# cpmech/russell

Measured on AMD Instinct MI355X. Metric: factorize+solve time (ms) + SpTRSV GB/s, 1M-DOF 5-pt Poisson f64, 1/2/4/8 GPU, lower is better.
Workload: dtype f64; 1 GPU; values+rhs resident in HBM: numeric LU factorize + solve, 2D 5-point Poisson 1000x1000 grid (n=1000000, nnz=4996000) f64, general storage, 1 RHS per GPU (through host pointers: value_host_boundary_ms); rhs_per_gpu=1, refinement_steps=1

## Files before the change

include/russell_hipmf.h:

```cpp
#ifndef RUSSELL_HIPMF_H
#define RUSSELL_HIPMF_H

#include <inttypes.h>
#include <stddef.h>

#ifdef __cplusplus
extern "C" {
#endif

#define C_BOOL int32_t

#define SUCCESSFUL_EXIT 0
#define ERROR_NULL_POINTER 100000
#define ERROR_MALLOC 200000
#define ERROR_VERSION 300000
#define ERROR_NOT_AVAILABLE 400000
#define ERROR_NEED_INITIALIZATION 500000
#define ERROR_NEED_FACTORIZATION 600000
#define ERROR_ALREADY_INITIALIZED 700000

#define HIPMF_WARNING_SINGULAR_MATRIX 1
#define ERROR_HIP_MALLOC 100
#define ERROR_HIP_MEMCPY 200
#define ERROR_HIP_SYNCHRONIZE 300
// ... 34 lines not shown

int32_t solver_hipmf_factorize(struct InterfaceHIPMF *solver,
                               int32_t *effective_ordering,
                               int32_t *effective_scaling,
                               int32_t *num_perturbed_pivots,
                               double *rcond_estimate,
                               double *determinant_coefficient,
                               double *determinant_exponent,
                               C_BOOL compute_determinant,
                               C_BOOL verbose,
                               const double *values);

int32_t solver_hipmf_solve(struct InterfaceHIPMF *solver, double *x, const double *rhs, C_BOOL verbose);


int32_t solver_hipmf_solve_many(struct InterfaceHIPMF *solver, double *x, const double *rhs, int32_t nrhs, int32_t ld,
                                C_BOOL verbose);

int32_t solver_hipmf_prepare_solve_many(struct InterfaceHIPMF *solver, int32_t nrhs);

int32_t solver_hipmf_factorize_device(struct InterfaceHIPMF *solver, const double *d_values);
int32_t solver_hipmf_solve_device(struct InterfaceHIPMF *solver, double *d_x, const double *d_rhs, int32_t nrhs, int32_t ld);

int32_t solver_hipmf_solve_transpose(struct InterfaceHIPMF *solver, double *x, const double *rhs, C_BOOL verbose);
int32_t solver_hipmf_solve_transpose_device(struct InterfaceHIPMF *solver, double *d_x, const double *d_rhs, int32_t nrhs, int32_t ld);
int32_t solver_hipmf_solve_transpose_many(struct InterfaceHIPMF *solver, double *x, const double *rhs, int32_t nrhs, int32_t ld, C_BOOL verbose);
int32_t solver_hipmf_solve_transpose_many_device(struct InterfaceHIPMF *solver, double *d_x, const double *d_rhs, int32_t nrhs, int32_t ld);

int32_t solver_hipmf_solve_sparse(struct InterfaceHIPMF *solver, double *x_sel, int32_t ldx, int32_t nrhs, const int32_t *rhs_ptr,
                                  const int32_t *rhs_idx, const double *rhs_val, int32_t nsel, const int32_t *sel_idx, C_BOOL verbose);
int32_t solver_hipmf_solve_sparse_device(struct InterfaceHIPMF *solver, double *d_x_sel, int32_t ldx, int32_t nrhs, const int32_t *d_rhs_ptr,
                                         const int32_t *d_rhs_idx, const double *d_rhs_val, int32_t nsel, const int32_t *d_sel_idx, C_BOOL verbose);
int32_t solver_hipmf_inverse_entries(struct InterfaceHIPMF *solver, int32_t nent, const int32_t *rows, const int32_t *cols, double *values, C_BOOL verbose);

int32_t solver_hipmf_solve_with_error_analysis(struct InterfaceHIPMF *solver, double *x, const double *rhs, double *error_analysis_array_len_8,
                                               int32_t error_analysis_option, C_BOOL verbose);

int32_t solver_hipmf_mat_vec_mul(struct InterfaceHIPMF *solver, double *v, double alpha, const double *u);

int32_t solver_hipmf_set_value_map(struct InterfaceHIPMF *solver, int32_t nnz_in, const int32_t *seg_ptr, const int32_t *seg_idx);
int32_t solver_hipmf_factorize_mapped(struct InterfaceHIPMF *solver, int32_t *effective_ordering, int32_t *effective_scaling,
                                      int32_t *num_perturbed_pivots, double *rcond_estimate, double *determinant_coefficient,
                                      double *determinant_exponent, C_BOOL compute_determinant, C_BOOL verbose,
                                      const double *input_values);
int32_t solver_hipmf_factorize_mapped_device(struct InterfaceHIPMF *solver, const double *d_input_values);

int32_t solver_hipmf_get_permutation(struct InterfaceHIPMF *solver, int32_t *perm);

int32_t hipmf_max_product_matching(int32_t ndim, const int32_t *row_pointers, const int32_t *col_indices, const double *values,
                                   int32_t *matched_row, double *row_scale, double *col_scale);
int32_t hipmf_paired_matching(int32_t ndim2, const int32_t *row_pointers, const int32_t *col_indices, const double *values, int32_t *matched_row,
                              double *row_scale, double *col_scale);

int32_t solver_hipmf_get_stats(struct InterfaceHIPMF *solver, int64_t *istats, double *dstats);
int32_t solver_hipmf_reset_timers(struct InterfaceHIPMF *solver);
#define HIPMF_COUNTER_REMATCH 0
#define HIPMF_COUNTER_WEAK_DIAGONAL_ROWS 1
#define HIPMF_COUNTER_FUSED_FALLBACKS 2
#define HIPMF_COUNTER_PERSISTENT_BYTES 3
#define HIPMF_COUNTER_ARENA_BYTES 4
#define HIPMF_COUNTER_SYMMETRIC_LDLT 5
#define HIPMF_COUNTER_SYM_EXPANDED 6
#define HIPMF_COUNTER_MID_FRONTS 8
#define HIPMF_COUNTER_CHAIN_FALLBACKS 7
#define HIPMF_COUNTER_PLAN_DIGEST 9
#define HIPMF_COUNTER_TAGGED_SOLVE 10
#define HIPMF_COUNTER_GATE_WAITS 11
#define HIPMF_COUNTER_WAVE_FRONTS 12
#define HIPMF_COUNTER_LEAF_FRONTS 13
#define HIPMF_COUNTER_SPLIT_SLABS 14
#define HIPMF_COUNTER_EVENT_FENCE_FREE 15
#define HIPMF_COUNTER_BLOCK_GROUPS 16
#define HIPMF_COUNTER_SYM_WEAK_DIAGONAL 17
#define HIPMF_COUNTER_BCAST_SLICED_BYTES 18
#define HIPMF_COUNTER_KRYLOV_ITERATIONS 19
#define HIPMF_COUNTER_TRANSPOSED_SOLVES 20
#define HIPMF_COUNTER_ANALYSIS_SOLVES 21
#define HIPMF_COUNTER_TRANSPOSED_KRYLOV_ITERATIONS 22
#define HIPMF_COUNTER_TRANSPOSED_BLOCKS 23
#define HIPMF_COUNTER_PRUNED_FWD_FRONTS 24
#define HIPMF_COUNTER_PRUNED_BWD_FRONTS 25
#define HIPMF_COUNTER_PRUNED_BLOCKS 26
#define HIPMF_COUNTER_PRUNED_BYTES 27
int64_t solver_hipmf_get_counter(struct InterfaceHIPMF *solver, int32_t which);

#define HIPMF_OPTION_MATCHING 0
#define HIPMF_OPTION_PIVOTING 1
#define HIPMF_OPTION_HYBRID_MEMORY 2
#define HIPMF_OPTION_ERROR_ESTIMATES 3
#define HIPMF_OPTION_CONDITION_NUMBERS 4
#define HIPMF_OPTION_SYM_RECHECK 5
#define HIPMF_OPTION_EFFECTIVE_PIVOTING 6
int32_t solver_hipmf_set_option(struct InterfaceHIPMF *solver, int32_t option, double value);
int32_t solver_hipmf_get_option(struct InterfaceHIPMF *solver, int32_t option, double *value);

#define HIPMF_COMM_ID_BYTES 128
int32_t solver_hipmf_factor_parts(struct InterfaceHIPMF *solver, int32_t max_parts, void **d_ptrs, int64_t *bytes);
int32_t hipmf_comm_unique_id(void *id128);
int32_t hipmf_comm_init_rank(void **comm, int32_t nranks, const void *id128, int32_t rank);
void hipmf_comm_destroy(void *comm);
int32_t solver_hipmf_broadcast_factor(struct InterfaceHIPMF *solver, void *comm, int32_t root, int32_t rank, double *seconds,
                                      int64_t *bytes_sent);
int32_t solver_hipmf_solve_many_sharded(struct InterfaceHIPMF *solver, double *d_x, const double *d_rhs, int32_t nrhs_total, int32_t ld,
                                        int32_t nranks, int32_t rank, int32_t *first_column, int32_t *num_columns);
int32_t solver_hipmf_adopt_factor(struct InterfaceHIPMF *solver, const double *d_values);

const char *solver_hipmf_last_error(struct InterfaceHIPMF *solver);

struct InterfaceComplexHIPMF;
struct InterfaceComplexHIPMF *complex_solver_hipmf_new(void);
void complex_solver_hipmf_drop(struct InterfaceComplexHIPMF *solver);
int32_t complex_solver_hipmf_initialize(struct InterfaceComplexHIPMF *solver, int32_t ordering, int32_t scaling, double pivot_epsilon,
                                        int32_t refinement_nstep, C_BOOL verbose, C_BOOL general_symmetric, int32_t ndim,
                                        const int32_t *row_pointers, const int32_t *col_indices, const double *values);
int32_t complex_solver_hipmf_factorize(struct InterfaceComplexHIPMF *solver, int32_t *effective_ordering, int32_t *effective_scaling,
                                       int32_t *num_perturbed_pivots, double *rcond_estimate, double *determinant_coefficient_real,
                                       double *determinant_coefficient_imag, double *determinant_exponent, C_BOOL compute_determinant, C_BOOL verbose,
                                       const double *values);
int32_t complex_solver_hipmf_get_determinant(struct InterfaceComplexHIPMF *solver, double *determinant_coefficient_real,
                                             double *determinant_coefficient_imag, double *determinant_exponent);
int32_t complex_solver_hipmf_solve(struct InterfaceComplexHIPMF *solver, double *x, const double *rhs, C_BOOL verbose);
int32_t complex_solver_hipmf_solve_transpose(struct InterfaceComplexHIPMF *solver, double *x, const double *rhs, int32_t conjugate, C_BOOL verbose);
int32_t complex_solver_hipmf_solve_with_error_analysis(struct InterfaceComplexHIPMF *solver, double *x, const double *rhs, double *error_analysis_array_len_8,
                                                       int32_t error_analysis_option, C_BOOL verbose);
int32_t complex_solver_hipmf_set_value_map(struct InterfaceComplexHIPMF *solver, int32_t nnz_in, const int32_t *seg_ptr, const int32_t *seg_idx);
int32_t complex_solver_hipmf_factorize_mapped(struct InterfaceComplexHIPMF *solver, int32_t *effective_ordering, int32_t *effective_scaling,
                                              int32_t *num_perturbed_pivots, double *rcond_estimate, C_BOOL verbose, const double *input_values);
int32_t complex_solver_hipmf_get_stats(struct InterfaceComplexHIPMF *solver, int64_t *istats, double *dstats);
int64_t complex_solver_hipmf_get_counter(struct InterfaceComplexHIPMF *solver, int32_t which);
const char *complex_solver_hipmf_last_error(struct InterfaceComplexHIPMF *solver);

void *hipmf_device_malloc(size_t bytes);
void hipmf_device_free(void *ptr);
int32_t hipmf_memcpy_h2d(void *dst, const void *src, size_t bytes);
int32_t hipmf_memcpy_d2h(void *dst, const void *src, size_t bytes);
int32_t hipmf_device_synchronize(void);
int32_t hipmf_device_count(void);
int32_t hipmf_device_mem_info(size_t *free_bytes, size_t *total_bytes);
int32_t hipmf_device_copy_bandwidth(int64_t bytes, int32_t reps, double *gb_per_s);
int32_t hipmf_device_mfma_rate(int32_t workgroups, int32_t iters, double *tflops);
int32_t hipmf_set_device(int32_t device);

void *hipmf_fdm_new(int32_t nx, int32_t ny, int32_t nz, int32_t periodic_x, int32_t periodic_y, int32_t periodic_z, int32_t sym,
                    const uint8_t *prescribed);
void hipmf_fdm_drop(void *fdm);
int32_t hipmf_fdm_dims(const void *fdm, int64_t *nu, int64_t *np, int64_t *nnz_bar, int64_t *nnz_check);
int32_t hipmf_fdm_structure_device(const void *fdm, int32_t *d_bar_i, int32_t *d_bar_j, int32_t *d_check_i, int32_t *d_check_j);
int32_t hipmf_fdm_values_device(const void *fdm, double dx, double dy, double dz, double kx, double ky, double kz, double alpha,
                                double *d_bar_values, double *d_check_values);
int32_t hipmf_fdm_lmm_dims(void *fdm, int64_t *neq, int64_t *nlag, int64_t *nnz);
int32_t hipmf_fdm_lmm_structure_device(void *fdm, int32_t *d_i, int32_t *d_j);
int32_t hipmf_fdm_lmm_values_device(void *fdm, double dx, double dy, double dz, double kx, double ky, double kz, double alpha, double *d_values);

#ifdef __cplusplus
}
#endif
#endif
```

russell_amd/_capi.py:

```python
import ctypes as C
import os

import numpy as np

_HERE = os.path.dirname(os.path.abspath(__file__))
DEFAULT_LIB = os.path.join(_HERE, "lib", "librussell_hipmf.so")

i32p = np.ctypeslib.ndpointer(dtype=np.int32, flags="C_CONTIGUOUS")
i64p = np.ctypeslib.ndpointer(dtype=np.int64, flags="C_CONTIGUOUS")
f64p = np.ctypeslib.ndpointer(dtype=np.float64, flags="C_CONTIGUOUS")

SYMBOLS = {
    "solver_hipmf_new": (C.c_void_p, []),
    "solver_hipmf_drop": (None, [C.c_void_p]),
    "solver_hipmf_initialize": (C.c_int32, [C.c_void_p, C.c_int32, C.c_int32, C.c_double, C.c_int32, C.c_int32, C.c_int32,
                                            C.c_int32, C.c_int32, i32p, i32p, C.c_void_p]),
    "solver_hipmf_factorize": (C.c_int32, [C.c_void_p, C.POINTER(C.c_int32), C.POINTER(C.c_int32), C.POINTER(C.c_int32),
                                           C.POINTER(C.c_double), C.POINTER(C.c_double), C.POINTER(C.c_double), C.c_int32,
                                           C.c_int32, f64p]),
    "solver_hipmf_solve": (C.c_int32, [C.c_void_p, f64p, f64p, C.c_int32]),
    "solver_hipmf_solve_many": (C.c_int32, [C.c_void_p, f64p, f64p, C.c_int32, C.c_int32, C.c_int32]),
    "solver_hipmf_prepare_solve_many": (C.c_int32, [C.c_void_p, C.c_int32]),
    "solver_hipmf_factorize_device": (C.c_int32, [C.c_void_p, C.c_void_p]),
    "solver_hipmf_solve_device": (C.c_int32, [C.c_void_p, C.c_void_p, C.c_void_p, C.c_int32, C.c_int32]),
    "solver_hipmf_solve_transpose": (C.c_int32, [C.c_void_p, f64p, f64p, C.c_int32]),
    "solver_hipmf_solve_transpose_device": (C.c_int32, [C.c_void_p, C.c_void_p, C.c_void_p, C.c_int32, C.c_int32]),
    "solver_hipmf_solve_transpose_many": (C.c_int32, [C.c_void_p, f64p, f64p, C.c_int32, C.c_int32, C.c_int32]),
    "solver_hipmf_solve_transpose_many_device": (C.c_int32, [C.c_void_p, C.c_void_p, C.c_void_p, C.c_int32, C.c_int32]),
    "solver_hipmf_solve_sparse": (C.c_int32, [C.c_void_p, f64p, C.c_int32, C.c_int32, i32p, i32p, f64p, C.c_int32, C.c_void_p, C.c_int32]),
    "solver_hipmf_solve_sparse_device": (C.c_int32, [C.c_void_p, C.c_void_p, C.c_int32, C.c_int32, C.c_void_p, C.c_void_p, C.c_void_p, C.c_int32,
                                                      C.c_void_p, C.c_int32]),
    "solver_hipmf_inverse_entries": (C.c_int32, [C.c_void_p, C.c_int32, i32p, i32p, f64p, C.c_int32]),
    "solver_hipmf_solve_with_error_analysis": (C.c_int32, [C.c_void_p, f64p, f64p, f64p, C.c_int32, C.c_int32]),
    "solver_hipmf_mat_vec_mul": (C.c_int32, [C.c_void_p, f64p, C.c_double, f64p]),
    "solver_hipmf_get_permutation": (C.c_int32, [C.c_void_p, i32p]),
    "solver_hipmf_set_value_map": (C.c_int32, [C.c_void_p, C.c_int32, i32p, i32p]),
    "solver_hipmf_factorize_mapped": (C.c_int32, [C.c_void_p, C.POINTER(C.c_int32), C.POINTER(C.c_int32), C.POINTER(C.c_int32),
                                                  C.POINTER(C.c_double), C.POINTER(C.c_double), C.POINTER(C.c_double), C.c_int32,
                                                  C.c_int32, f64p]),
    "solver_hipmf_factorize_mapped_device": (C.c_int32, [C.c_void_p, C.c_void_p]),
    "hipmf_max_product_matching": (C.c_int32, [C.c_int32, i32p, i32p, f64p, i32p, f64p, f64p]),
    "hipmf_paired_matching": (C.c_int32, [C.c_int32, i32p, i32p, f64p, i32p, f64p, f64p]),
    "solver_hipmf_get_stats": (C.c_int32, [C.c_void_p, i64p, f64p]),
    "solver_hipmf_reset_timers": (C.c_int32, [C.c_void_p]),
    "complex_solver_hipmf_new": (C.c_void_p, []),
    "complex_solver_hipmf_drop": (None, [C.c_void_p]),
    "complex_solver_hipmf_initialize": (C.c_int32, [C.c_void_p, C.c_int32, C.c_int32, C.c_double, C.c_int32, C.c_int32, C.c_int32, C.c_int32,
                                                     i32p, i32p, C.c_void_p]),
    "complex_solver_hipmf_factorize": (C.c_int32, [C.c_void_p, C.POINTER(C.c_int32), C.POINTER(C.c_int32), C.POINTER(C.c_int32),
                                                    C.POINTER(C.c_double), C.POINTER(C.c_double), C.POINTER(C.c_double), C.POINTER(C.c_double),
                                                    C.c_int32, C.c_int32, f64p]),
    "complex_solver_hipmf_get_determinant": (C.c_int32, [C.c_void_p, C.POINTER(C.c_double), C.POINTER(C.c_double), C.POINTER(C.c_double)]),
    "complex_solver_hipmf_solve": (C.c_int32, [C.c_void_p, f64p, f64p, C.c_int32]),
    "complex_solver_hipmf_solve_transpose": (C.c_int32, [C.c_void_p, f64p, f64p, C.c_int32, C.c_int32]),
    "complex_solver_hipmf_solve_with_error_analysis": (C.c_int32, [C.c_void_p, f64p, f64p, f64p, C.c_int32, C.c_int32]),
    "complex_solver_hipmf_set_value_map": (C.c_int32, [C.c_void_p, C.c_int32, i32p, i32p]),
    "complex_solver_hipmf_factorize_mapped": (C.c_int32, [C.c_void_p, C.POINTER(C.c_int32), C.POINTER(C.c_int32), C.POINTER(C.c_int32),
                                                           C.POINTER(C.c_double), C.c_int32, f64p]),
    "complex_solver_hipmf_get_stats": (C.c_int32, [C.c_void_p, i64p, f64p]),
    "complex_solver_hipmf_get_counter": (C.c_int64, [C.c_void_p, C.c_int32]),
    "complex_solver_hipmf_last_error": (C.c_char_p, [C.c_void_p]),
    "solver_hipmf_get_counter": (C.c_int64, [C.c_void_p, C.c_int32]),
    "solver_hipmf_set_option": (C.c_int32, [C.c_void_p, C.c_int32, C.c_double]),
    "solver_hipmf_get_option": (C.c_int32, [C.c_void_p, C.c_int32, C.POINTER(C.c_double)]),
    "solver_hipmf_factor_parts": (C.c_int32, [C.c_void_p, C.c_int32, C.POINTER(C.c_void_p), C.POINTER(C.c_int64)]),
    "hipmf_comm_unique_id": (C.c_int32, [C.c_void_p]),
    "hipmf_comm_init_rank": (C.c_int32, [C.POINTER(C.c_void_p), C.c_int32, C.c_void_p, C.c_int32]),
    "hipmf_comm_destroy": (None, [C.c_void_p]),
    "solver_hipmf_broadcast_factor": (C.c_int32, [C.c_void_p, C.c_void_p, C.c_int32, C.c_int32, C.POINTER(C.c_double), C.POINTER(C.c_int64)]),
    "solver_hipmf_solve_many_sharded": (C.c_int32, [C.c_void_p, C.c_void_p, C.c_void_p, C.c_int32, C.c_int32, C.c_int32, C.c_int32,
                                                     C.POINTER(C.c_int32), C.POINTER(C.c_int32)]),
    "solver_hipmf_adopt_factor": (C.c_int32, [C.c_void_p, C.c_void_p]),
    "solver_hipmf_last_error": (C.c_char_p, [C.c_void_p]),
    "hipmf_device_malloc": (C.c_void_p, [C.c_size_t]),
    "hipmf_device_free": (None, [C.c_void_p]),
    "hipmf_memcpy_h2d": (C.c_int32, [C.c_void_p, C.c_void_p, C.c_size_t]),
    "hipmf_memcpy_d2h": (C.c_int32, [C.c_void_p, C.c_void_p, C.c_size_t]),
    "hipmf_device_synchronize": (C.c_int32, []),
    "hipmf_device_count": (C.c_int32, []),
    "hipmf_device_copy_bandwidth": (C.c_int32, [C.c_int64, C.c_int32, C.POINTER(C.c_double)]),
    "hipmf_device_mem_info": (C.c_int32, [C.POINTER(C.c_size_t), C.POINTER(C.c_size_t)]),
    "hipmf_device_mfma_rate": (C.c_int32, [C.c_int32, C.c_int32, C.POINTER(C.c_double)]),
    "hipmf_set_device": (C.c_int32, [C.c_int32]),
    "hipmf_fdm_new": (C.c_void_p, [C.c_int32, C.c_int32, C.c_int32, C.c_int32, C.c_int32, C.c_int32, C.c_int32, C.c_void_p]),
    "hipmf_fdm_drop": (None, [C.c_void_p]),
    "hipmf_fdm_dims": (C.c_int32, [C.c_void_p, C.POINTER(C.c_int64), C.POINTER(C.c_int64), C.POINTER(C.c_int64), C.POINTER(C.c_int64)]),
    "hipmf_fdm_structure_device": (C.c_int32, [C.c_void_p, C.c_void_p, C.c_void_p, C.c_void_p, C.c_void_p]),
    "hipmf_fdm_values_device": (C.c_int32, [C.c_void_p, C.c_double, C.c_double, C.c_double, C.c_double, C.c_double, C.c_double, C.c_double,
                                            C.c_void_p, C.c_void_p]),
    "hipmf_fdm_lmm_dims": (C.c_int32, [C.c_void_p, C.POINTER(C.c_int64), C.POINTER(C.c_int64), C.POINTER(C.c_int64)]),
    "hipmf_fdm_lmm_structure_device": (C.c_int32, [C.c_void_p, C.c_void_p, C.c_void_p]),
    "hipmf_fdm_lmm_values_device": (C.c_int32, [C.c_void_p, C.c_double, C.c_double, C.c_double, C.c_double, C.c_double, C.c_double, C.c_double, C.c_void_p]),
}

_cache = {}


def load(path=None):
    path = path or os.environ.get("HIPMF_DEV_LIB") or DEFAULT_LIB
    if path in _cache:
        return _cache[path]
    if not os.path.exists(path):
        raise RuntimeError(
            "russell_amd: %s is missing -- build the HIP extension first (python -c 'import __graft_entry__ as g; g.build()'). "
            "There is no CPU fallback." % path)
    lib = C.CDLL(path)
    for name, (res, args) in SYMBOLS.items():
        fn = getattr(lib, name)
        fn.restype = res
        fn.argtypes = args
    _cache[path] = lib
    return lib
```

russell_amd/backend.py:

```python
import ctypes as C

import numpy as np

from . import _capi

ISTAT_NAMES = ["ndim", "nnz_a", "nsuper", "nlevels", "nnz_l", "nnz_u", "max_front", "max_pivots", "n_perturbed", "n_zero_pivot",
               "refinement_steps", "factor_launches", "solve_launches", "pool_bytes", "matched", "fused_fallbacks"]
DSTAT_NAMES = ["flops", "flops_gemm", "ordering_s", "symbolic_s", "assemble_ms", "factor_ms", "fwd_ms", "bwd_ms", "solve_total_ms",
               "residual_inf", "acc_assemble_ms", "acc_factor_ms", "acc_factor_count", "acc_fwd_ms", "acc_bwd_ms", "acc_tri_count"]


class HipmfError(RuntimeError):
    def __init__(self, code, where, detail=""):
        super().__init__("%s failed with status %d %s" % (where, code, detail))
        self.code = code


class Hipmf:
    def __init__(self, lib_path=None):
        self.lib = _capi.load(lib_path)
        self.h = self.lib.solver_hipmf_new()
        if not self.h:
            raise RuntimeError("solver_hipmf_new returned NULL: no HIP device visible (there is no CPU fallback)")
        self.n = 0
# ... 70 lines not shown
    def solve_with_error_analysis(self, rhs, option, verbose=False, array=None):
        b = np.ascontiguousarray(rhs, dtype=np.float64)
        x = np.zeros(self.n)
        ea = np.zeros(8) if array is None else array
        code = self.lib.solver_hipmf_solve_with_error_analysis(self.h, x, b, ea, int(option), int(verbose))
        if code != 0:
            raise self._err(code, "solver_hipmf_solve_with_error_analysis")
        return x, ea

    def solve_many(self, rhs_colmajor, ld=None):
        b = np.ascontiguousarray(rhs_colmajor, dtype=np.float64)
        ld = self.n if ld is None else int(ld)
        if b.ndim != 2 or b.shape[1] != ld:
            raise ValueError("solve_many expects an array of shape (nrhs, ld) with ld = %d, got %r" % (ld, b.shape))
        nrhs = b.shape[0]
        x = np.zeros_like(b)
        x[:, self.n:] = b[:, self.n:]
        code = self.lib.solver_hipmf_solve_many(self.h, x, b, nrhs, ld, 0)
        if code != 0:
            raise self._err(code, "solver_hipmf_solve_many")
        return x

    def solve_transpose_many(self, rhs_colmajor, ld=None):
        b = np.ascontiguousarray(rhs_colmajor, dtype=np.float64)
        ld = self.n if ld is None else int(ld)
        if b.ndim != 2 or b.shape[1] != ld:
            raise ValueError("solve_transpose_many expects an array of shape (nrhs, ld) with ld = %d, got %r" % (ld, b.shape))
        nrhs = b.shape[0]
        x = np.zeros_like(b)
        x[:, self.n:] = b[:, self.n:]
        code = self.lib.solver_hipmf_solve_transpose_many(self.h, x, b, nrhs, ld, 0)
        if code != 0:
            raise self._err(code, "solver_hipmf_solve_transpose_many")
        return x

    def solve_sparse(self, rhs_ptr, rhs_idx, rhs_val, select=None, ldx=None, verbose=False):
        ptr = np.ascontiguousarray(rhs_ptr, dtype=np.int32)
        idx = np.ascontiguousarray(rhs_idx, dtype=np.int32)
        val = np.ascontiguousarray(rhs_val, dtype=np.float64)
        nrhs = int(ptr.size) - 1
        sel = None if select is None else np.ascontiguousarray(select, dtype=np.int32)
        nsel = self.n if sel is None else int(sel.size)
        ldx = nsel if ldx is None else int(ldx)
        x = np.zeros((max(nrhs, 0), max(ldx, 0)))
        code = self.lib.solver_hipmf_solve_sparse(self.h, x, ldx, nrhs, ptr, idx, val, nsel, None if sel is None else sel.ctypes.data, int(verbose))
        if code != 0:
            raise self._err(code, "solver_hipmf_solve_sparse")
        return x

    def inverse_entries(self, rows, cols, verbose=False):
        r = np.ascontiguousarray(rows, dtype=np.int32)
        c = np.ascontiguousarray(cols, dtype=np.int32)
        if r.shape != c.shape or r.ndim != 1:
            raise ValueError("inverse_entries expects two index vectors of equal length, got %r and %r" % (r.shape, c.shape))
        v = np.zeros(r.size)
        code = self.lib.solver_hipmf_inverse_entries(self.h, int(r.size), r, c, v, int(verbose))
        if code != 0:
            raise self._err(code, "solver_hipmf_inverse_entries")
        return v

    def mat_vec_mul(self, u, alpha=1.0):
        v = np.zeros(self.n)
        code = self.lib.solver_hipmf_mat_vec_mul(self.h, v, alpha, np.ascontiguousarray(u, dtype=np.float64))
        if code != 0:
            raise self._err(code, "solver_hipmf_mat_vec_mul")
        return v

    def permutation(self):
        p = np.zeros(self.n, np.int32)
        code = self.lib.solver_hipmf_get_permutation(self.h, p)
        if code != 0:
            raise self._err(code, "solver_hipmf_get_permutation")
        return p

    def stats(self):
        i, d = np.zeros(16, np.int64), np.zeros(16)
        code = self.lib.solver_hipmf_get_stats(self.h, i, d)
        if code != 0:
            raise self._err(code, "solver_hipmf_get_stats")
        out = {k: int(v) for k, v in zip(ISTAT_NAMES, i)}
        out.update({k: float(v) for k, v in zip(DSTAT_NAMES, d)})
        return out

    COUNTERS = {"rematch": 0, "weak_diagonal_rows": 1, "fused_fallbacks": 2, "persistent_bytes": 3, "arena_bytes": 4, "symmetric_ldlt": 5, "sym_expanded": 6, "chain_fallbacks": 7, "mid_fronts": 8, "plan_digest": 9, "tagged_solve": 10, "gate_waits": 11, "wave_fronts": 12, "leaf_fronts": 13, "split_slabs": 14, "event_fence_free": 15, "block_groups": 16, "sym_weak_diagonal": 17, "bcast_sliced_bytes": 18, "krylov_iterations": 19, "transposed_solves": 20, "analysis_solves": 21, "transposed_krylov_iterations": 22, "transposed_blocks": 23, "pruned_fwd_fronts": 24, "pruned_bwd_fronts": 25, "pruned_blocks": 26, "pruned_bytes": 27}

    OPTIONS = {"matching": 0, "pivoting": 1, "hybrid_memory": 2, "error_estimates": 3, "condition_numbers": 4, "sym_recheck": 5}

    def set_option(self, name, value):
        return int(self.lib.solver_hipmf_set_option(self.h, self.OPTIONS[name], float(value)))

    def counter(self, name):
        return int(self.lib.solver_hipmf_get_counter(self.h, self.COUNTERS[name]))

    def reset_timers(self):
        self.lib.solver_hipmf_reset_timers(self.h)

    def dev_alloc(self, nbytes):
        p = self.lib.hipmf_device_malloc(nbytes)
        if not p:
            raise MemoryError("hipmf_device_malloc(%d)" % nbytes)
        return p

    def dev_free(self, p):
        self.lib.hipmf_device_free(p)

    def h2d(self, dptr, arr):
        a = np.ascontiguousarray(arr)
        code = self.lib.hipmf_memcpy_h2d(dptr, a.ctypes.data_as(C.c_void_p), a.nbytes)
        if code != 0:
            raise self._err(code, "hipmf_memcpy_h2d")

    def d2h(self, arr, dptr):
        assert arr.flags["C_CONTIGUOUS"]
        code = self.lib.hipmf_memcpy_d2h(arr.ctypes.data_as(C.c_void_p), dptr, arr.nbytes)
        if code != 0:
            raise self._err(code, "hipmf_memcpy_d2h")

    def factorize_device(self, d_values):
        return self.lib.solver_hipmf_factorize_device(self.h, d_values)

    def factorize_mapped_device(self, d_input_values):
        return self.lib.solver_hipmf_factorize_mapped_device(self.h, d_input_values)

    def factor_buffers(self):
        ptrs = (C.c_void_p * 4)()
        sizes = (C.c_int64 * 4)()
        k = self.lib.solver_hipmf_factor_parts(self.h, 4, ptrs, sizes)
        if k != 4:
            raise self._err(k, "solver_hipmf_factor_parts")
        return [(int(ptrs[i] or 0), int(sizes[i])) for i in range(4)]

    def broadcast_factor(self, comm, root, rank):
        sec, nb = C.c_double(0.0), C.c_int64(0)
        code = self.lib.solver_hipmf_broadcast_factor(self.h, comm, root, rank, C.byref(sec), C.byref(nb))
        if code != 0:
            raise self._err(code, "solver_hipmf_broadcast_factor")
        return sec.value, nb.value

    def solve_many_sharded(self, d_x, d_rhs, nrhs_total, nranks, rank, ld=None):
        first, count = C.c_int32(0), C.c_int32(0)
        code = self.lib.solver_hipmf_solve_many_sharded(self.h, d_x, d_rhs, nrhs_total, ld or self.n, nranks, rank, C.byref(first), C.byref(count))
        if code != 0:
            raise self._err(code, "solver_hipmf_solve_many_sharded")
        return first.value, count.value

    def adopt_factor(self, d_values):
        return self.lib.solver_hipmf_adopt_factor(self.h, d_values)

    def prepare_solve_many(self, nrhs):
        code = self.lib.solver_hipmf_prepare_solve_many(self.h, int(nrhs))
        if code != 0:
            raise self._err(code, "solver_hipmf_prepare_solve_many")

    def solve_device(self, d_x, d_rhs, nrhs=1, ld=None):
        code = self.lib.solver_hipmf_solve_device(self.h, d_x, d_rhs, nrhs, ld or self.n)
        if code != 0:
            raise self._err(code, "solver_hipmf_solve_device")

    def solve_transpose_device(self, d_x, d_rhs, nrhs=1, ld=None):
        code = self.lib.solver_hipmf_solve_transpose_device(self.h, d_x, d_rhs, nrhs, ld or self.n)
        if code != 0:
            raise self._err(code, "solver_hipmf_solve_transpose_device")

    def solve_transpose_many_device(self, d_x, d_rhs, nrhs, ld=None):
        code = self.lib.solver_hipmf_solve_transpose_many_device(self.h, d_x, d_rhs, nrhs, ld or self.n)
        if code != 0:
            raise self._err(code, "solver_hipmf_solve_transpose_many_device")
# ... 6 lines not shown
```

russell_amd/csrc/interface_complex_hipmf.cpp:

```cpp
#include <hipmf_device_rt.h>

#include <algorithm>
#include <cstdio>
#include <new>
#include <string>
#include <vector>

#include "numeric.hpp"
#include "../../include/russell_hipmf.h"

using namespace hipmf;

struct InterfaceComplexHIPMF {
    Solver solver;
    int32_t n = 0;
    int64_t nnz = 0;
    bool sym_lower = false;
    std::vector<int32_t> src_entry;
    std::vector<int8_t> src_code;
    int32_t effective_ordering = 0;
    bool triplet_map = false;
    int8_t pairs_state = 0;
};

// ... 211 lines not shown
int32_t complex_solver_hipmf_factorize_mapped(struct InterfaceComplexHIPMF *h, int32_t *effective_ordering, int32_t *effective_scaling,
                                              int32_t *num_perturbed_pivots, double *rcond_estimate, C_BOOL verbose, const double *input_values) {
    return guarded(h, [&]() { return c_factorize_mapped_body(h, effective_ordering, effective_scaling, num_perturbed_pivots, rcond_estimate, verbose, input_values); });
}

int32_t complex_solver_hipmf_get_determinant(struct InterfaceComplexHIPMF *h, double *determinant_coefficient_real, double *determinant_coefficient_imag,
                                             double *determinant_exponent) {
    if (!h) return ERROR_NULL_POINTER;
    return guarded(h, [&]() { return h->solver.determinant_complex(determinant_coefficient_real, determinant_coefficient_imag, determinant_exponent, nullptr); });
}

static int32_t c_solve_body(struct InterfaceComplexHIPMF *h, double *x, const double *rhs, C_BOOL verbose) {
    if (!h || !x || !rhs) return ERROR_NULL_POINTER;
    if (!h->solver.factorized) return ERROR_NEED_FACTORIZATION;
    h->solver.opt.verbose = verbose == 1;
    return h->solver.solve(x, rhs, 1, 2 * (int64_t)h->n, false);
}

int32_t complex_solver_hipmf_solve(struct InterfaceComplexHIPMF *h, double *x, const double *rhs, C_BOOL verbose) {
    return guarded(h, [&]() { return c_solve_body(h, x, rhs, verbose); });
}

int32_t complex_solver_hipmf_solve_transpose(struct InterfaceComplexHIPMF *h, double *x, const double *rhs, int32_t conjugate, C_BOOL verbose) {
    return guarded(h, [&]() {
        if (!h || !x || !rhs) return (int32_t)ERROR_NULL_POINTER;
        if (!h->solver.factorized) return (int32_t)ERROR_NEED_FACTORIZATION;
        if (conjugate != 0 && conjugate != 1) return (int32_t)ERROR_HIPMF_INVALID_VALUE;
        h->solver.opt.verbose = verbose == 1;
        return h->solver.solve_transpose(x, rhs, 1, h->solver.S.n, false, conjugate == 0);
    });
}

static int32_t check_pairs(struct InterfaceComplexHIPMF *h) {
    if (h->pairs_state == 0) {
        std::vector<int32_t> rp, ci;
        const int32_t code = h->solver.download_pattern(rp, ci);
        if (code != SUCCESSFUL_EXIT) return code;
        bool ok = rp.size() == (size_t)2 * h->n + 1 && ci.size() == h->src_code.size();
        for (int32_t i = 0; ok && i < h->n; i++)
            for (int32_t q = rp[(size_t)2 * i]; ok && q < rp[(size_t)2 * i + 1]; q += 2)
                ok = q + 1 < rp[(size_t)2 * i + 1] && (ci[(size_t)q] & 1) == 0 && ci[(size_t)q + 1] == ci[(size_t)q] + 1 && h->src_code[(size_t)q] == 0 &&
                     h->src_code[(size_t)q + 1] == 1 && h->src_entry[(size_t)q] == h->src_entry[(size_t)q + 1];
        h->pairs_state = ok ? 1 : -1;
    }
    if (h->pairs_state > 0) return SUCCESSFUL_EXIT;
    h->solver.last_error = "internal error: the real-equivalent rows 2i do not hold complex entries as adjacent (re, -im) pairs";
    return ERROR_HIPMF_SYMBOLIC;
}

int32_t complex_solver_hipmf_solve_with_error_analysis(struct InterfaceComplexHIPMF *h, double *x, const double *rhs, double *error_analysis_array_len_8,
                                                       int32_t error_analysis_option, C_BOOL verbose) {
    return guarded(h, [&]() {
        if (!h || !x || !rhs || !error_analysis_array_len_8) return (int32_t)ERROR_NULL_POINTER;
        if (!h->solver.factorized) return (int32_t)ERROR_NEED_FACTORIZATION;
        if (error_analysis_option < 0 || error_analysis_option > 2) return (int32_t)ERROR_HIPMF_INVALID_VALUE;
        int32_t code = error_analysis_option == 0 ? (int32_t)SUCCESSFUL_EXIT : check_pairs(h);
        if (code != SUCCESSFUL_EXIT) return code;
        code = c_solve_body(h, x, rhs, verbose);
        if (code != SUCCESSFUL_EXIT) return code;
        return h->solver.error_analysis_complex(x, rhs, error_analysis_array_len_8, error_analysis_option);
    });
}

const char *complex_solver_hipmf_last_error(struct InterfaceComplexHIPMF *h) { return h ? h->solver.last_error.c_str() : "null solver"; }

static int32_t c_get_stats_body(struct InterfaceComplexHIPMF *h, int64_t *is, double *ds) {
    if (!h || !is || !ds) return ERROR_NULL_POINTER;
    if (!h->solver.initialized) return ERROR_NEED_INITIALIZATION;
    const Solver &s = h->solver;
    for (int i = 0; i < 16; i++) is[i] = 0, ds[i] = 0.0;
    is[0] = h->n, is[1] = h->nnz, is[2] = s.S.nsuper, is[3] = s.S.nlevels, is[4] = s.S.nnz_l, is[5] = s.S.nnz_u, is[6] = s.S.max_front;
    is[7] = s.S.max_pivots, is[8] = s.n_perturbed, is[9] = s.n_zero_pivot, is[10] = s.refinement_steps_done;
    is[11] = s.times.n_kernel_launches_factor, is[12] = s.times.n_kernel_launches_solve, is[13] = s.pool_doubles * 8, is[14] = s.matched ? 1 : 0;
    is[15] = s.fused_fallbacks;
    ds[0] = s.S.flops, ds[1] = s.S.flops_gemm, ds[2] = s.S.seconds_ordering, ds[3] = s.S.seconds_total, ds[4] = s.times.scale_assemble_ms;
    ds[5] = s.times.factor_ms, ds[6] = s.times.fwd_ms, ds[7] = s.times.bwd_ms, ds[8] = s.times.solve_total_ms, ds[9] = s.last_residual_inf;
    return SUCCESSFUL_EXIT;
}

int32_t complex_solver_hipmf_get_stats(struct InterfaceComplexHIPMF *h, int64_t *is, double *ds) {
    return guarded(h, [&]() { return c_get_stats_body(h, is, ds); });
}

int64_t complex_solver_hipmf_get_counter(struct InterfaceComplexHIPMF *h, int32_t which) {
    if (!h || !h->solver.initialized) return -1;
    const Solver &s = h->solver;
    switch (which) {
    case HIPMF_COUNTER_REMATCH: return s.rematch_count;
    case HIPMF_COUNTER_WEAK_DIAGONAL_ROWS: return s.n_weak_diag;
    case HIPMF_COUNTER_FUSED_FALLBACKS: return s.fused_fallbacks;
    case HIPMF_COUNTER_PERSISTENT_BYTES: return s.S.persist_doubles * 8;
    case HIPMF_COUNTER_ARENA_BYTES: return s.S.temp_doubles * 8;
    case HIPMF_COUNTER_SYMMETRIC_LDLT: return s.S.sym_mode ? 1 : 0;
    case HIPMF_COUNTER_CHAIN_FALLBACKS: return s.chain_fallbacks;
    case HIPMF_COUNTER_MID_FRONTS: return s.mid_front_count;
    case HIPMF_COUNTER_TAGGED_SOLVE: return s.tagged_solve() ? 1 : 0;
    case HIPMF_COUNTER_GATE_WAITS: return s.gate_waits;
    case HIPMF_COUNTER_WAVE_FRONTS: return s.wave_front_count;
    case HIPMF_COUNTER_LEAF_FRONTS: return s.leaf_front_count();
    case HIPMF_COUNTER_SPLIT_SLABS: return s.split_slab_count();
    case HIPMF_COUNTER_KRYLOV_ITERATIONS: return s.krylov_iterations;
    case HIPMF_COUNTER_TRANSPOSED_SOLVES: return s.transposed_solves;
    case HIPMF_COUNTER_ANALYSIS_SOLVES: return s.analysis_solves;
    case HIPMF_COUNTER_TRANSPOSED_KRYLOV_ITERATIONS: return s.krylov_iterations_t;
    default: return -1;
    }
}

}
```

russell_amd/csrc/interface_hipmf.cpp:

```cpp
#include <hipmf_device_rt.h>

#include <algorithm>
#include <chrono>
#include <cstdio>
#include <cstring>
#include <mutex>
#include <new>
#ifdef HIPMF_HAVE_RCCL
#include <dlfcn.h>
#include <rccl/rccl.h>
#endif

#include "numeric.hpp"
#include "matching.hpp"
#include "../../include/russell_hipmf.h"

using namespace hipmf;

struct InterfaceHIPMF {
    Solver solver;
    int32_t ordering_requested = 0;
    int32_t effective_ordering = 0;
    int32_t opt_matching = 1, opt_pivoting = 0, opt_sym_recheck = 0;
    int64_t bcast_sliced_bytes = 0;
// ... 482 lines not shown

int32_t hipmf_max_product_matching(int32_t ndim, const int32_t *row_pointers, const int32_t *col_indices, const double *values,
                                   int32_t *matched_row, double *row_scale, double *col_scale) {
    if (!row_pointers || !col_indices || !values || !matched_row || !row_scale || !col_scale) return ERROR_NULL_POINTER;
    if (ndim < 1 || validate_csr(ndim, row_pointers, col_indices) != 0) return ERROR_HIPMF_INVALID_MATRIX;
    std::vector<int32_t> mrow;
    std::vector<double> dr, dc;
    if (max_product_matching(ndim, row_pointers, col_indices, values, mrow, dr, dc) != 0) return ERROR_HIPMF_INVALID_MATRIX;
    for (int32_t i = 0; i < ndim; i++) matched_row[i] = mrow[i], row_scale[i] = dr[i], col_scale[i] = dc[i];
    return SUCCESSFUL_EXIT;
}

int32_t hipmf_paired_matching(int32_t ndim2, const int32_t *row_pointers, const int32_t *col_indices, const double *values, int32_t *matched_row,
                              double *row_scale, double *col_scale) {
    if (!row_pointers || !col_indices || !values || !matched_row || !row_scale || !col_scale) return ERROR_NULL_POINTER;
    if (ndim2 < 2 || ndim2 % 2 != 0 || validate_csr(ndim2, row_pointers, col_indices) != 0) return ERROR_HIPMF_INVALID_MATRIX;
    return guarded(nullptr, [&]() {
        std::vector<int32_t> mrow;
        std::vector<double> dr, dc;
        if (paired_matching(ndim2, row_pointers, col_indices, values, mrow, dr, dc) != 0) return (int32_t)ERROR_HIPMF_INVALID_MATRIX;
        for (int32_t i = 0; i < ndim2; i++) matched_row[i] = mrow[i], row_scale[i] = dr[i], col_scale[i] = dc[i];
        return (int32_t)SUCCESSFUL_EXIT;
    });
}

int32_t solver_hipmf_get_permutation(struct InterfaceHIPMF *h, int32_t *perm) {
    if (!h || !perm) return ERROR_NULL_POINTER;
    if (!h->solver.initialized) return ERROR_NEED_INITIALIZATION;
    for (int32_t i = 0; i < h->solver.S.n; i++) perm[i] = h->solver.S.perm[i];
    return SUCCESSFUL_EXIT;
}

int32_t solver_hipmf_get_stats(struct InterfaceHIPMF *h, int64_t *is, double *ds) {
    if (!h || !is || !ds) return ERROR_NULL_POINTER;
    if (!h->solver.initialized) return ERROR_NEED_INITIALIZATION;
    const Solver &s = h->solver;
    for (int i = 0; i < 16; i++) is[i] = 0, ds[i] = 0.0;
    is[0] = s.S.n, is[1] = s.S.nnz_a, is[2] = s.S.nsuper, is[3] = s.S.nlevels, is[4] = s.S.nnz_l, is[5] = s.S.nnz_u;
    is[6] = s.S.max_front, is[7] = s.S.max_pivots, is[8] = s.n_perturbed, is[9] = s.n_zero_pivot;
    is[10] = s.refinement_steps_done, is[11] = s.times.n_kernel_launches_factor, is[12] = s.times.n_kernel_launches_solve;
    is[13] = s.pool_doubles * 8;
    is[14] = s.matched ? 1 : 0;
    is[15] = s.fused_fallbacks;
    ds[0] = s.S.flops, ds[1] = s.S.flops_gemm, ds[2] = s.S.seconds_ordering, ds[3] = s.S.seconds_total;
    ds[4] = s.times.scale_assemble_ms, ds[5] = s.times.factor_ms, ds[6] = s.times.fwd_ms, ds[7] = s.times.bwd_ms;
    ds[8] = s.times.solve_total_ms, ds[9] = s.last_residual_inf;
    ds[10] = s.times.acc_assemble_ms, ds[11] = s.times.acc_factor_ms, ds[12] = (double)s.times.acc_factor_count;
    ds[13] = s.times.acc_fwd_ms, ds[14] = s.times.acc_bwd_ms, ds[15] = (double)s.times.acc_tri_count;
    return SUCCESSFUL_EXIT;
}

int64_t solver_hipmf_get_counter(struct InterfaceHIPMF *h, int32_t which) {
    if (!h || !h->solver.initialized) return -1;
    const Solver &s = h->solver;
    switch (which) {
    case HIPMF_COUNTER_REMATCH: return s.rematch_count;
    case HIPMF_COUNTER_WEAK_DIAGONAL_ROWS: return s.n_weak_diag;
    case HIPMF_COUNTER_FUSED_FALLBACKS: return s.fused_fallbacks;
    case HIPMF_COUNTER_PERSISTENT_BYTES: return s.S.persist_doubles * 8;
    case HIPMF_COUNTER_ARENA_BYTES: return s.S.temp_doubles * 8;
    case HIPMF_COUNTER_SYMMETRIC_LDLT: return s.S.sym_mode ? 1 : 0;
    case HIPMF_COUNTER_SYM_EXPANDED: return h->expanded ? 1 : 0;
    case HIPMF_COUNTER_CHAIN_FALLBACKS: return s.chain_fallbacks;
    case HIPMF_COUNTER_MID_FRONTS: return s.mid_front_count;
    case HIPMF_COUNTER_PLAN_DIGEST: return s.plan_digest;
    case HIPMF_COUNTER_TAGGED_SOLVE: return s.tagged_solve() ? 1 : 0;
    case HIPMF_COUNTER_GATE_WAITS: return s.gate_waits;
    case HIPMF_COUNTER_WAVE_FRONTS: return s.wave_front_count;
    case HIPMF_COUNTER_LEAF_FRONTS: return s.leaf_front_count();
    case HIPMF_COUNTER_SPLIT_SLABS: return s.split_slab_count();
    case HIPMF_COUNTER_EVENT_FENCE_FREE: return s.event_fence_free ? 1 : 0;
    case HIPMF_COUNTER_BLOCK_GROUPS: return s.block_groups_last;
    case HIPMF_COUNTER_SYM_WEAK_DIAGONAL: return s.sym_weak_diag_seen ? 1 : 0;
    case HIPMF_COUNTER_BCAST_SLICED_BYTES: return h->bcast_sliced_bytes;
    case HIPMF_COUNTER_KRYLOV_ITERATIONS: return s.krylov_iterations;
    case HIPMF_COUNTER_TRANSPOSED_SOLVES: return s.transposed_solves;
    case HIPMF_COUNTER_ANALYSIS_SOLVES: return s.analysis_solves;
    case HIPMF_COUNTER_TRANSPOSED_KRYLOV_ITERATIONS: return s.krylov_iterations_t;
    case HIPMF_COUNTER_TRANSPOSED_BLOCKS: return s.transposed_blocks;
    case HIPMF_COUNTER_PRUNED_FWD_FRONTS: return s.pruned_fwd_fronts;
    case HIPMF_COUNTER_PRUNED_BWD_FRONTS: return s.pruned_bwd_fronts;
    case HIPMF_COUNTER_PRUNED_BLOCKS: return s.pruned_blocks;
    case HIPMF_COUNTER_PRUNED_BYTES: return s.pruned_bytes;
    default: return -1;
    }
}

int32_t solver_hipmf_factor_parts(struct InterfaceHIPMF *h, int32_t max_parts, void **d_ptrs, int64_t *bytes) {
    if (!h || !d_ptrs || !bytes) return ERROR_NULL_POINTER;
    if (!h->solver.initialized) return ERROR_NEED_INITIALIZATION;
    const Solver &s = h->solver;
    void *p[4] = {s.d_pool, s.d_lperm, s.d_rs, s.d_diag_ptr()};
    const int64_t nb[4] = {s.S.persist_doubles * 8, (int64_t)s.S.n * 4, (int64_t)s.S.n * 8, (int64_t)s.S.n * 8};
    if (max_parts < 4) return ERROR_HIPMF_INVALID_VALUE;
    for (int i = 0; i < 4; i++) d_ptrs[i] = p[i], bytes[i] = nb[i];
    return 4;
}

int32_t solver_hipmf_adopt_factor(struct InterfaceHIPMF *h, const double *d_values) {
    if (!h || !d_values) return ERROR_NULL_POINTER;
    if (!h->solver.initialized) return ERROR_NEED_INITIALIZATION;
    return guarded(h, [&]() { return h->solver.adopt_factor(d_values); });
}

int32_t solver_hipmf_reset_timers(struct InterfaceHIPMF *h) {
    if (!h) return ERROR_NULL_POINTER;
    PhaseTimes &t = h->solver.times;
    t.acc_assemble_ms = t.acc_factor_ms = t.acc_fwd_ms = t.acc_bwd_ms = 0.0;
    t.acc_factor_count = t.acc_tri_count = 0;
    return SUCCESSFUL_EXIT;
}

#ifdef HIPMF_HAVE_RCCL
namespace {
struct Rccl {
    void *dl = nullptr;
    decltype(&ncclGetUniqueId) get_unique_id = nullptr;
    decltype(&ncclCommInitRank) comm_init_rank = nullptr;
    decltype(&ncclCommDestroy) comm_destroy = nullptr;
    decltype(&ncclBroadcast) broadcast = nullptr;
    decltype(&ncclAllReduce) all_reduce = nullptr;
    decltype(&ncclSend) send = nullptr;
    decltype(&ncclRecv) recv = nullptr;
    decltype(&ncclGroupStart) group_start = nullptr;
    decltype(&ncclGroupEnd) group_end = nullptr;
    decltype(&ncclCommCount) comm_count = nullptr;
    bool tried = false, ok = false;
    bool p2p() const { return send && recv && group_start && group_end && comm_count; }
};
Rccl g_rccl;
std::mutex g_rccl_mutex;
bool rccl_load() {
    std::lock_guard<std::mutex> lock(g_rccl_mutex);
    if (g_rccl.tried) return g_rccl.ok;
    g_rccl.tried = true;
    for (const char *name : {"librccl.so.1", "librccl.so", "/opt/rocm/lib/librccl.so.1"}) {
        g_rccl.dl = dlopen(name, RTLD_NOW | RTLD_GLOBAL);
        if (g_rccl.dl) break;
    }
    if (!g_rccl.dl) return false;
    g_rccl.get_unique_id = (decltype(g_rccl.get_unique_id))dlsym(g_rccl.dl, "ncclGetUniqueId");
    g_rccl.comm_init_rank = (decltype(g_rccl.comm_init_rank))dlsym(g_rccl.dl, "ncclCommInitRank");
    g_rccl.comm_destroy = (decltype(g_rccl.comm_destroy))dlsym(g_rccl.dl, "ncclCommDestroy");
    g_rccl.broadcast = (decltype(g_rccl.broadcast))dlsym(g_rccl.dl, "ncclBroadcast");
    g_rccl.all_reduce = (decltype(g_rccl.all_reduce))dlsym(g_rccl.dl, "ncclAllReduce");
    g_rccl.send = (decltype(g_rccl.send))dlsym(g_rccl.dl, "ncclSend");
    g_rccl.recv = (decltype(g_rccl.recv))dlsym(g_rccl.dl, "ncclRecv");
    g_rccl.group_start = (decltype(g_rccl.group_start))dlsym(g_rccl.dl, "ncclGroupStart");
    g_rccl.group_end = (decltype(g_rccl.group_end))dlsym(g_rccl.dl, "ncclGroupEnd");
    g_rccl.comm_count = (decltype(g_rccl.comm_count))dlsym(g_rccl.dl, "ncclCommCount");
    g_rccl.ok = g_rccl.get_unique_id && g_rccl.comm_init_rank && g_rccl.comm_destroy && g_rccl.broadcast && g_rccl.all_reduce;
    return g_rccl.ok;
}
}

int32_t hipmf_comm_unique_id(void *id128) {
    if (!id128) return ERROR_NULL_POINTER;
    if (!rccl_load()) return ERROR_NOT_AVAILABLE;
    static_assert(sizeof(ncclUniqueId) == HIPMF_COMM_ID_BYTES, "ncclUniqueId size");
    return g_rccl.get_unique_id((ncclUniqueId *)id128) == ncclSuccess ? SUCCESSFUL_EXIT : ERROR_HIPMF_COMM;
}

int32_t hipmf_comm_init_rank(void **comm, int32_t nranks, const void *id128, int32_t rank) {
    if (!comm || !id128) return ERROR_NULL_POINTER;
    if (nranks < 1 || rank < 0 || rank >= nranks) return ERROR_HIPMF_INVALID_VALUE;
    if (!rccl_load()) return ERROR_NOT_AVAILABLE;
// ... 230 lines not shown
```

russell_amd/csrc/kernels.hpp:

```cpp
#pragma once
#include "kernels_assembly.hpp"
#include "kernels_common.hpp"
#include "kernels_factor.hpp"
#include "kernels_extend_add.hpp"
#include "kernels_factor_front.hpp"
#include "kernels_factor_binv.hpp"
#include "kernels_solve.hpp"
#include "kernels_solve_fused.hpp"
#include "kernels_factor_chain.hpp"
#include "kernels_solve_tree.hpp"
#include "kernels_solve_leaf.hpp"
#include "kernels_vector.hpp"
```

russell_amd/csrc/kernels_factor.hpp:

```cpp
#pragma once
#include "kernels_common.hpp"

namespace hipmf {

constexpr int LU_KB = 8;
template <int NW, bool PIVOT, bool PAIRED = false>
__device__ __forceinline__ void lds_lu_blocked(double *__restrict__ S, const int ld, const int f, const int p, int32_t *lp, int32_t *pivpos,
                                               const double eps, const double rep, FactorInfo *info, double *zd = nullptr) {
    constexpr int KB = LU_KB, T = 64 * NW;
    const int lin = threadIdx.x, lane = lin & 63, wave = lin >> 6;
    for (int c0 = 0; c0 < p; c0 += KB) {
        const int kb = (p - c0) < KB ? (p - c0) : KB;
        if (wave == 0) {
            const int r = lane;
            const bool active = r >= c0 && r < f;
            double a[KB];
#pragma unroll
            for (int q = 0; q < KB; q++) a[q] = (active && q < kb) ? S[r + (c0 + q) * ld] : 0.0;
            int pos = r;
            bool chosen = false;
            int npert = 0, nzero = 0;
            const int lp_old = (PIVOT && r >= c0 && r < p) ? lp[r] : 0;
            int pv_prev = 0;
#pragma unroll
// ... 74 lines not shown
            }
        }
        __syncthreads();
        const int R0 = c0 + kb;
        if (R0 >= f) break;
        for (int col = R0 + lin; col < f; col += T) {
            double x[KB];
#pragma unroll
            for (int t = 0; t < KB; t++) x[t] = (t < kb) ? S[(c0 + t) + col * ld] : 0.0;
#pragma unroll
            for (int t = 1; t < KB; t++) {
                if (t < kb) {
#pragma unroll
                    for (int q = 0; q < t; q++) x[t] -= S[(c0 + t) + (c0 + q) * ld] * x[q];
                }
            }
#pragma unroll
            for (int t = 1; t < KB; t++)
                if (t < kb) S[(c0 + t) + col * ld] = x[t];
        }
        __syncthreads();
        {
            const int nt = (f - R0 + 15) >> 4, ntot = nt * nt;
            const int l15 = lane & 15, l4 = lane >> 4;
            const int ka = l4 < kb ? l4 : kb - 1, kb2 = 4 + l4 < kb ? 4 + l4 : kb - 1;
            const bool k0ok = l4 < kb, k1ok = 4 + l4 < kb;
            auto tile_load = [&](int ti, int tj, double &a0, double &a1, double &b0, double &b1, f64x4 &acc) {
                const int rA = R0 + 16 * ti + l15, cB = R0 + 16 * tj + l15;
                const int rAc = rA < f ? rA : f - 1, cBc = cB < f ? cB : f - 1;
                a0 = S[rAc + (c0 + ka) * ld], a1 = S[rAc + (c0 + kb2) * ld];
                b0 = S[(c0 + ka) + cBc * ld], b1 = S[(c0 + kb2) + cBc * ld];
#pragma unroll
                for (int g = 0; g < 4; g++) {
                    const int rr = R0 + 16 * ti + l4 + 4 * g;
                    acc[g] = S[(rr < f ? rr : f - 1) + cBc * ld];
                }
                if (rA >= f || !k0ok) a0 = 0.0;
                if (rA >= f || !k1ok) a1 = 0.0;
                if (cB >= f || !k0ok) b0 = 0.0;
                if (cB >= f || !k1ok) b1 = 0.0;
            };
            auto tile_store = [&](int ti, int tj, const f64x4 &acc) {
                const int cB = R0 + 16 * tj + l15;
#pragma unroll
                for (int g = 0; g < 4; g++) {
                    const int rr = R0 + 16 * ti + l4 + 4 * g;
                    if (rr < f && cB < f) S[rr + cB * ld] = acc[g];
                }
            };
            int ti = wave % nt, tj = wave / nt;
            for (int tile = wave; tile < ntot; tile += 2 * NW) {
                int ti2 = ti + NW, tj2 = tj;
                while (ti2 >= nt) ti2 -= nt, tj2++;
                const bool two = tile + NW < ntot;
                double a0, a1, b0, b1, c0a, c1a, d0, d1;
                f64x4 acc, acc2;
                tile_load(ti, tj, a0, a1, b0, b1, acc);
                if (two) tile_load(ti2, tj2, c0a, c1a, d0, d1, acc2);
                acc = mfma_f64_16x16x4(-a0, b0, acc);
                acc = mfma_f64_16x16x4(-a1, b1, acc);
                if (two) {
                    acc2 = mfma_f64_16x16x4(-c0a, d0, acc2);
                    acc2 = mfma_f64_16x16x4(-c1a, d1, acc2);
                }
                tile_store(ti, tj, acc);
                if (two) tile_store(ti2, tj2, acc2);
                ti = ti2 + NW, tj = tj2;
                while (ti >= nt) ti -= nt, tj++;
            }
        }
        __syncthreads();
    }
}

struct SmallAsm {
    const SmallDesc *sd;
    const int32_t *sa_k;
    const uint16_t *sa_pos;
    const double *vs, *vs2;
    const int32_t *child_idx, *rel;
    const int32_t *list0;
};

template <int NW, bool PAIRED = false>
__global__ void __launch_bounds__(64 * NW, NW == 1 ? 6 : 2) k_small_factor(const int32_t *__restrict__ list, const FrontDesc *__restrict__ FD,
                                                          double *__restrict__ pool, int32_t *__restrict__ lperm,
                                                          const unsigned long long *__restrict__ anorm_bits, double pivot_eps,
                                                          FactorInfo *info, int32_t ld, SmallAsm A, double *__restrict__ diag) {
    HIPMF_DYN_SHARED(double, sm);
    __shared__ int32_t lp[SMALL_F];
    __shared__ int32_t pivpos[LU_KB];
    const int tid = threadIdx.x & 63, grp = threadIdx.x >> 6;
    const int lin = threadIdx.x;
    const SmallDesc sdesc = A.sd[(list - A.list0) + blockIdx.x];
    const FrontDesc fd = sdesc.fd;
    const int p = fd.p, f = fd.p + fd.m;
    double *F = pool + fd.off;
    const double eps = pivot_eps * __longlong_as_double((long long)*anorm_bits);
    const double rep = pivot_replacement(pivot_eps, __longlong_as_double((long long)*anorm_bits));
    const int nch = fd.child_end - fd.child_begin;
    int64_t d_cb = 0, d_ldc = 0, d_rel = 0;
    int d_m = 0;
    if (grp == 0 && tid < nch) {
        const FrontDesc cd = FD[A.child_idx[fd.child_begin + tid]];
        d_ldc = cd.ld;
        d_cb = cd.off + cd.p + (int64_t)cd.p * cd.ld;
        d_rel = cd.rowptr;
        d_m = cd.m;
    }
    const int e0 = sdesc.e0, e1 = sdesc.e1;
    for (int e = lin; e < f * ld; e += 64 * NW) sm[e] = 0.0;
    __syncthreads();
    for (int e = e0 + lin; e < e1; e += 64 * NW) {
        const int kk = A.sa_k[e];
        const int pos = A.sa_pos[e];
        const double v = kk < 0 ? A.vs2[~kk] : A.vs[kk];
        sm[(pos & 255) + (pos >> 8) * ld] = v;
    }
    __syncthreads();
    if (grp == 0) {
        for (int c0 = 0; c0 < nch; c0 += 64) {
            if (c0 > 0) {
                d_m = 0;
                if (c0 + tid < nch) {
                    const FrontDesc cd = FD[A.child_idx[fd.child_begin + c0 + tid]];
                    d_ldc = cd.ld;
                    d_cb = cd.off + cd.p + (int64_t)cd.p * cd.ld;
                    d_rel = cd.rowptr;
                    d_m = cd.m;
                }
            }
            const int nbatch = nch - c0 < 64 ? nch - c0 : 64;
            if (nch > 64 && __ballot(d_m > 1) == 0ull) {
                const int myq = (tid < nbatch && d_m == 1) ? A.rel[d_rel] : -1;
                const double myv = myq >= 0 ? pool[d_cb] : 0.0;
                for (int l = 0; l < nbatch; l++) {
                    const int q = wave_bcast_i32(myq, l);
                    const double v = wave_bcast(myv, l);
                    if (tid == 0 && q >= 0) sm[q + q * ld] += v;
                }
                wave_sync();
                continue;
            }
            for (int cl = 0; cl < nbatch; cl++) {
                const int64_t cbo = wave_bcast_i64(d_cb, cl), ldc = wave_bcast_i64(d_ldc, cl), relo = wave_bcast_i64(d_rel, cl);
                const int mc = wave_bcast_i32(d_m, cl);
                if (mc == 0) continue;
                const double *CB = pool + cbo;
                const int sh = mc <= 16 ? 4 : (mc <= 32 ? 5 : 6);
                const int i = tid & ((1 << sh) - 1), g = tid >> sh, G = 64 >> sh;
                const int myrel = i < mc ? A.rel[relo + i] : 0;
                for (int jb = 0; jb < mc; jb += 16 * G) {
                    double cb[16];
#pragma unroll
                    for (int q = 0; q < 16; q++) {
                        const int j = jb + g + q * G;
                        cb[q] = (i < mc && j < mc) ? CB[i + (int64_t)j * ldc] : 0.0;
                    }
#pragma unroll
                    for (int q = 0; q < 16; q++) {
                        const int j = jb + g + q * G;
                        const int rj = __shfl(myrel, j & 63);
                        if (i < mc && j < mc) sm[myrel + rj * ld] += cb[q];
                    }
                }
                wave_sync();
            }
        }
        if (tid < p) lp[tid] = tid;
    }
    __syncthreads();
    if constexpr (PAIRED) lds_lu_blocked<NW, true, true>(sm, ld, f, p, lp, pivpos, eps, rep, info, reinterpret_cast<const FactorInfoExt *>(info)->zdiag + fd.first);
    else lds_lu_blocked<NW, true>(sm, ld, f, p, lp, pivpos, eps, rep, info);
    const bool split = fd.epoff >= 0;
    if (tid < f) {
        int c = grp;
        for (; c + 7 * NW < f; c += 8 * NW) {
            double a[8];
#pragma unroll
            for (int q = 0; q < 8; q++) a[q] = sm[tid + (c + q * NW) * ld];
#pragma unroll
            for (int q = 0; q < 8; q++) F[tid + (c + q * NW) * f] = (split && c + q * NW < p && tid <= c + q * NW) ? 0.0 : a[q];
        }
        for (; c < f; c += NW) F[tid + c * f] = (split && c < p && tid <= c) ? 0.0 : sm[tid + c * ld];
    }
    if (split && tid < p) {
        double *Up = pool + fd.epoff;
        for (int c = grp; c < f; c += NW) Up[tid + c * p] = (tid > c) ? 0.0 : sm[tid + c * ld];
    }
    if (grp == 0 && tid < p) {
        lperm[fd.first + tid] = lp[tid];
        diag[fd.first + tid] = sm[tid + tid * ld];
    }
}

template <bool PIVOT = true, bool PAIRED = false>
__device__ __forceinline__ void tile_lu32_z(double (&a)[NB], int lane, double eps, double rep, int &step, int &npert, int &nzero, double &zr, double &zi) {
    step = -1;
    npert = 0;
    nzero = 0;
    int pv_prev = 0;
#pragma clang loop unroll(full)
    for (int c = 0; c < NB; c++) {
        const bool cand = lane < NB && step < 0;
        const unsigned mag = __float_as_uint((float)fabs(a[c]));
        const unsigned key = cand ? ((mag & ~63u) | 32u | (unsigned)(31 - lane)) : 0u;
        const double myinv = fast_rcp(a[c]);
        int pv;
        if constexpr (PAIRED) pv = (c & 1) ? (pv_prev ^ 1) : 31 - (int)(wave_max_u32<2>(key) & 31u);
        else pv = PIVOT ? 31 - (int)(wave_max_u32<2>(key) & 31u) : c;
        pv_prev = pv;
        if (lane == pv) step = c;
        double d = wave_bcast(a[c], pv);
        double inv = wave_bcast(myinv, pv);
        if (fabs(d) < eps || d == 0.0) {
            double dn = (d < 0.0) ? -rep : rep;
            if (dn == 0.0) dn = 1.0;
            if (lane == pv) a[c] = dn;
            npert++;
            if (d == 0.0) nzero++;
            inv = 1.0 / dn;
            d = dn;
        }
        if constexpr (PAIRED) {
            if ((c & 1) == 0) {
                const double q = wave_bcast(a[c], pv ^ 1);
                if (lane == pv) zr = (pv & 1) ? q : d, zi = (pv & 1) ? d : q;
            }
        }
        const bool below = lane < NB && step < 0;
        if (below) a[c] *= inv;
        const double lmul = below ? a[c] : 0.0;
#pragma clang loop unroll(full)
        for (int cc = c + 1; cc < NB; cc++) a[cc] -= lmul * wave_bcast(a[cc], pv);
    }
}
template <bool PIVOT = true> __device__ __forceinline__ void tile_lu32(double (&a)[NB], int lane, double eps, double rep, int &step, int &npert, int &nzero) {
    double zr, zi;
    tile_lu32_z<PIVOT, false>(a, lane, eps, rep, step, npert, nzero, zr, zi);
}

template <bool SYM, bool PAIRED = false>
__global__ void __launch_bounds__(64) k_diag0(const FrontDesc *__restrict__ LFD, double *__restrict__ pool, int32_t *__restrict__ lperm,
                                              double *__restrict__ dws, const unsigned long long *__restrict__ anorm_bits, double pivot_eps,
                                              FactorInfo *info, double *__restrict__ diag) {
    const int slot = blockIdx.x, tid = threadIdx.x;
    FrontDesc fd = LFD[slot];
    const int nb = fd.p < NB ? fd.p : NB;
    const double *F = pool + fd.off;
    const int64_t ld = fd.ld;
    double a[NB];
#pragma unroll
    for (int c = 0; c < NB; c++) {
        const int rr = (SYM && tid < c) ? c : tid, cc = (SYM && tid < c) ? tid : c;
        a[c] = (tid < nb && c < nb) ? F[rr + (int64_t)cc * ld] : (tid == c ? 1.0 : 0.0);
    }
    const double eps = pivot_eps * __longlong_as_double((long long)*anorm_bits);
    const double rep = pivot_replacement(pivot_eps, __longlong_as_double((long long)*anorm_bits));
    int step, npert, nzero;
    double zr = 0.0, zi = 0.0;
    tile_lu32_z<!SYM, PAIRED>(a, tid, eps, rep, step, npert, nzero, zr, zi);
    if (tid < nb) {
        double *dw = dws + (int64_t)slot * NB * NB;
        double dg = 1.0;
#pragma unroll
        for (int c = 0; c < NB; c++) {
            if (c < nb) dw[step + c * nb] = a[c];
            if (c == step) dg = a[c];
        }
        lperm[fd.first + step] = tid;
        diag[fd.first + step] = dg;
        store_zpivot<PAIRED>(info, fd.first, step, zr, zi);
    }
    if (tid == 0 && npert > 0) {
        atomicAdd(&info->n_perturbed, npert);
        if (nzero > 0) atomicAdd(&info->n_zero_pivot, nzero);
// ... 609 lines not shown
```

russell_amd/csrc/numeric.cpp:

```cpp
#include "numeric.hpp"

#include <algorithm>
#include <chrono>
#include <thread>
#include <cmath>
#include <cstdio>
#include <cstdlib>
#include <cstring>
#include <functional>
#include <mutex>

#include "kernels.hpp"
#include "kernels_solve_transpose.hpp"
#include "kernels_solve_transpose_blocked.hpp"
#include "kernels_solve_pruned.hpp"
#include "kernels_error_analysis_complex.hpp"
#include <fcntl.h>
#include <sys/mman.h>
#include <pthread.h>
#include <atomic>
#include <sys/stat.h>
#include <unistd.h>
#include <cerrno>
#include "matching.hpp"
// ... 147 lines not shown
        HIPC(hipMemcpy(d_rp, rp, sizeof(int32_t) * ((size_t)n + 1), hipMemcpyHostToDevice), ERROR_HIP_MALLOC);
        HIPC(d_ci.alloc((size_t)std::max<int64_t>(nnz, 1)), ERROR_HIP_MALLOC);
        if (nnz > 0) HIPC(hipMemcpy(d_ci, ci, sizeof(int32_t) * (size_t)nnz, hipMemcpyHostToDevice), ERROR_HIP_MALLOC);
        HIPC(d_arow.upload(h_arow), ERROR_HIP_MALLOC);
        if (sym_lower) {
            std::vector<int32_t> tptr((size_t)n + 1, 0), tidx;
            for (int64_t k = 0; k < nnz; k++)
                if (ci[k] != h_arow[k]) tptr[ci[k] + 1]++;
            for (int32_t i = 0; i < n; i++) tptr[i + 1] += tptr[i];
            tidx.resize((size_t)tptr[n]);
            std::vector<int32_t> w(tptr.begin(), tptr.end() - 1);
            for (int64_t k = 0; k < nnz; k++)
                if (ci[k] != h_arow[k]) tidx[w[ci[k]]++] = (int32_t)k;
            HIPC(d_tptr.upload(tptr), ERROR_HIP_MALLOC);
            HIPC(d_tidx.upload(tidx), ERROR_HIP_MALLOC);
        }
        return SUCCESSFUL_EXIT;
    };
    std::thread prep_thread([&]() {
        try {
            prep_code = prep();
        } catch (const std::bad_alloc &) {
            std::lock_guard<std::mutex> lock(err_mutex);
            last_error = "Not enough memory: a host allocation failed";
            prep_code = ERROR_MALLOC;
        } catch (...) {
            std::lock_guard<std::mutex> lock(err_mutex);
            last_error = "initialize: the device set-up failed with an exception";
            prep_code = ERROR_HIPMF_INVALID_VALUE;
        }
    });
    struct PrepJoiner {
        std::thread &t;
        ~PrepJoiner() {
            if (t.joinable()) t.join();
        }
    } prep_joiner{prep_thread};
    if (!rematching) {
        h_rp_keep.assign(rp, rp + n + 1);
        h_ci_keep.assign(ci, ci + rp[n]);
        sopt_keep = sopt;
        sym_lower_keep = sym_lower;
    }
    lap("validate + streams + keep");
    SymbolicOptions so = sopt;
    so.augment_above = SMALL_F;
    so.symmetric_ldlt = sym_lower;
    if (const char *e = getenv("HIPMF_SYM_LDLT")) so.symmetric_ldlt = sym_lower && atoi(e) != 0;
    if (opt.complex_pairs && (sym_lower || n % 2 != 0)) {
        last_error = "complex pairs need general storage and an even order";
        return ERROR_HIPMF_INVALID_MATRIX;
    }
    so.pair_blocks = opt.complex_pairs;
    so.nd_leaf = 16;
    so.dense_leaves = true;
    if (const char *e = getenv("HIPMF_ND_LEAF")) {
        int v = atoi(e);
        so.dense_leaves = v > 0;
        so.nd_leaf = v > 0 ? std::min(v, 64) : 64;
    }
    solve_lanes_auto = true;
    solve_lanes = 1, solve_lanes_auto = false;
    if (const char *e = getenv("HIPMF_SMALL_WIDE")) small_wide_max = atoi(e);
    if (const char *e = getenv("HIPMF_SMALL_SPLIT")) small_split = atoi(e);
    if (const char *e = getenv("HIPMF_UPD_G4")) upd_g4 = std::max(65, atoi(e));
    if (const char *e = getenv("HIPMF_UPD_G8")) upd_g8 = std::max(upd_g4, atoi(e));
    if (const char *e = getenv("HIPMF_UPD_G16")) upd_g16 = std::max(upd_g8, atoi(e));
    if (const char *e = getenv("HIPMF_SPLIT_PIVOTS")) so.split_pivots = std::max(0, atoi(e));
    if (const char *e = getenv("HIPMF_DENSE_ROWS")) so.dense_row_factor = atof(e);
    if (const char *e = getenv("HIPMF_ND_THREADS")) so.nd_threads = std::max(1, atoi(e));
    if (const char *e = getenv("HIPMF_PAR_MIN")) so.parallel_min_n = std::max(0, atoi(e));
    if (const char *e = getenv("HIPMF_RELAX")) {
        int a, b, c;
        double x, y, z;
        if (sscanf(e, "%d,%d,%d,%lf,%lf,%lf", &a, &b, &c, &x, &y, &z) == 6)
            so.relax_ncol[0] = a, so.relax_ncol[1] = b, so.relax_ncol[2] = c, so.relax_zeros[0] = x, so.relax_zeros[1] = y, so.relax_zeros[2] = z;
    }
    if (const char *e = getenv("HIPMF_RELAX_BIG")) so.relax_big_front = std::max(0, atoi(e));
    if (const char *e = getenv("HIPMF_PAR_CHUNK")) so.parallel_chunk_min = std::max(1, atoi(e));
    if (const char *e = getenv("HIPMF_FUSED_SOLVE")) use_fused = atoi(e) != 0;
    if (const char *e = getenv("HIPMF_OVERLAP_SMALL")) overlap_small = atoi(e) != 0;
    small_pair = false;
    if (const char *e = getenv("HIPMF_SMALL_PAIR")) small_pair = atoi(e) != 0;
    if (const char *e = getenv("HIPMF_TREE_SOLVE")) use_tree = atoi(e) != 0;
    if (const char *e = getenv("HIPMF_TAG_SOLVE")) use_tag = atoi(e) != 0;
    if (const char *e = getenv("HIPMF_LEAF_KERNELS")) leaf_kernels = atoi(e) != 0;
    if (const char *e = getenv("HIPMF_SPLIT_TASKS")) split_tasks = std::max(0, atoi(e));
    split_minlen_env = false;
    if (const char *e = getenv("HIPMF_SPLIT_MINLEN")) split_minlen = std::max(64, atoi(e)), split_minlen_env = true;
    if (const char *e = getenv("HIPMF_BLOCK_GROUPS_BYTES")) block_groups_max_bytes = atof(e);
    if (const char *e = getenv("HIPMF_PLAIN_BAND")) plain_band = atoi(e) != 0;
    if (const char *e = getenv("HIPMF_REARM_TAGS")) rearm_tags = atoi(e) != 0;
    if (const char *e = getenv("HIPMF_KRYLOV")) krylov_enabled = atoi(e) != 0;
    if (const char *e = getenv("HIPMF_KRYLOV_RESTART")) krylov_restart = std::max(4, atoi(e));
    if (const char *e = getenv("HIPMF_KRYLOV_TOL")) krylov_tol = atof(e);
    if (const char *e = getenv("HIPMF_KRYLOV_OMEGA")) krylov_omega_ok = atof(e);
    if (const char *e = getenv("HIPMF_WAVE_FRONTS")) wave_fronts = atoi(e) != 0;
    if (const char *e = getenv("HIPMF_WAVE_FRONTS_BWD")) wave_fronts_bwd = atoi(e) != 0;
    if (const char *e = getenv("HIPMF_HOST_DIRECT")) host_direct = atoi(e) != 0;
    if (const char *e = getenv("HIPMF_MID_BWD_LEN4")) mid_bwd_len4 = std::max(1, atoi(e));
    if (const char *e = getenv("HIPMF_MID_BWD_LEN5")) mid_bwd_len5 = std::max(1, atoi(e));
    if (const char *e = getenv("HIPMF_WT_FRONTS")) wt_max_fronts = std::max(1, atoi(e));
    if (const char *e = getenv("HIPMF_WT_KB")) wt_max_kb = std::max(1, atoi(e));
    if (const char *e = getenv("HIPMF_UP_STAGE")) up_stage = std::max(0, std::min(64, atoi(e) / 8 * 8));
    if (const char *e = getenv("HIPMF_UP_STAGE_BWD")) up_stage_bwd = std::max(8, std::min(64, atoi(e) / 8 * 8));
    if (const char *e = getenv("HIPMF_UP_TOP_FRONTS")) up_top_fronts = std::max(1, atoi(e));
    if (const char *e = getenv("HIPMF_UP_REPLICAS")) use_rep = atoi(e) != 0;
    if (const char *e = getenv("HIPMF_UP_PAIR_XCD")) up_pair_xcd = atoi(e) != 0;
    if (const char *e = getenv("HIPMF_UP_MAX_GROUPS")) up_max_groups = std::max(2, std::min(32, atoi(e)));
    blocked_slabs_env = false;
    if (const char *e = getenv("HIPMF_BLOCKED_SLABS")) blocked_slabs = atoi(e) != 0, blocked_slabs_env = true;
    if (const char *e = getenv("HIPMF_UP_STAGE_MID")) up_stage_mid = std::max(0, std::min(32, atoi(e) / 8 * 8));
    if (const char *e = getenv("HIPMF_SF_BIG_ROWS")) sf_big_rows = std::max(0, std::min(7, atoi(e)));
    if (const char *e = getenv("HIPMF_SF_BIG_FRONT")) sf_big_front = std::max(65, atoi(e));
    if (const char *e = getenv("HIPMF_SF_ASM_FRONT")) sf_asm_front = atoi(e);
    if (const char *e = getenv("HIPMF_FACTOR_CHAIN")) use_chain = atoi(e) != 0;
    if (const char *e = getenv("HIPMF_CHAIN_FINE")) chain_fine = atoi(e) != 0;
    if (const char *e = getenv("HIPMF_CHAIN_MAX_WGS")) chain_max_update = std::max(0, atoi(e));
    if (const char *e = getenv("HIPMF_CHAIN_MIN_WGS")) chain_min_update = std::max(0, atoi(e));
    if (const char *e = getenv("HIPMF_CHAIN_MAX_STEPS")) chain_max_steps = std::max(0, atoi(e));
    if (const char *e = getenv("HIPMF_UPD32_MAXF")) upd32_max_front = std::max(0, atoi(e));
    if (const char *e = getenv("HIPMF_FACTOR_GRAPH")) use_graph = atoi(e) != 0;
    if (const char *e = getenv("HIPMF_UPD_SPLIT")) upd_split_min = std::max(0, atoi(e));
    if (const char *e = getenv("HIPMF_BLOCK_INV")) use_binv = atoi(e) != 0;
    if (const char *e = getenv("HIPMF_EA_LDS")) use_ea_lds = atoi(e) != 0;
    if (const char *e = getenv("HIPMF_EA_LU")) use_ea_lu = atoi(e) != 0;
    if (const char *e = getenv("HIPMF_UPD_XCD")) upd_xcd = atoi(e) != 0;
    if (const char *e = getenv("HIPMF_MID_LU_SPLIT")) mid_lu_split = atoi(e) != 0;
    if (const char *e = getenv("HIPMF_MID_FRONT")) use_mid = atoi(e) != 0;
    if (const char *e = getenv("HIPMF_MID_MMAX")) mid_mmax = std::max(0, std::min(MID_MMAX, atoi(e)));
    if (const char *e = getenv("HIPMF_MID_LU")) use_mid_lu = atoi(e) != 0;
    if (const char *e = getenv("HIPMF_MID_LU_MMAX")) mid_lu_mmax = std::max(1, atoi(e));
    if (const char *e = getenv("HIPMF_DIAG0_MIN")) diag0_min_panels = atoi(e);
    if (const char *e = getenv("HIPMF_SOLVE_SLAB64")) slab64 = atoi(e) != 0;
    if (const char *e = getenv("HIPMF_MATCHING")) opt.matching = atoi(e);
    if (opt.complex_pairs) {
        use_chain = false, use_binv = false, mid_mmax = 0;
    }
    std::vector<int32_t> mrow, rpB, ciB;
    std::vector<int64_t> kB;
    std::vector<double> dr, dc;
    matched = false;
    if (values && !sym_lower && n > 1 && opt.matching > 0 && rp[0] == 0 && (opt.matching >= 2 || diagonal_is_weak(n, rp, ci, values, 0.01, opt.complex_pairs))) {
        if ((opt.complex_pairs ? paired_matching(n, rp, ci, values, mrow, dr, dc) : max_product_matching(n, rp, ci, values, mrow, dr, dc)) == 0) {
            matched = true;
            rpB.assign((size_t)n + 1, 0);
            for (int32_t j = 0; j < n; j++) rpB[j + 1] = rpB[j] + (rp[mrow[j] + 1] - rp[mrow[j]]);
            ciB.resize((size_t)rp[n]);
            kB.resize((size_t)rp[n]);
            for (int32_t j = 0; j < n; j++)
                for (int32_t p = rp[mrow[j]], q = rpB[j]; p < rp[mrow[j] + 1]; p++, q++) ciB[q] = ci[p], kB[p] = q;
            if (opt.verbose) fprintf(stderr, "hipmf: initialize: maximum-product matching + scaling applied (weak diagonal)\n");
        } else if (opt.verbose) {
            fprintf(stderr, "hipmf: initialize: the matrix has no perfect matching (structurally singular); continuing without\n");
        }
    }
    so.pool_limit_live = &live_pool_limit;
    lap("matching test");
    int rc = matched ? analyse(n, rpB.data(), ciB.data(), false, so, S) : analyse(n, rp, ci, sym_lower, so, S);
    lap("analyse");
    prep_thread.join();
    so.pool_limit_bytes = live_pool_limit.load();
    if (prep_code != SUCCESSFUL_EXIT) return prep_code;
    if (rc == 0 && so.pool_limit_bytes > 0.0 && S.pool_estimate_bytes > so.pool_limit_bytes) rc = -40;
    lap("wait for the device set-up");
    if (rc == -40) {
// ... 252 lines not shown
            uint64_t hsh = 1469598103934665603ull;
            auto mix = [&](uint64_t v) {
                for (int b = 0; b < 8; b++) hsh = (hsh ^ ((v >> (8 * b)) & 0xff)) * 1099511628211ull;
            };
            for (int32_t k = 0; k < n; k++) mix((uint64_t)(uint32_t)S.perm[k] | ((uint64_t)(matched ? (uint32_t)mrow[S.perm[k]] : 0u) << 32));
            mix((uint64_t)S.persist_doubles), mix((uint64_t)S.temp_doubles), mix((uint64_t)S.nsuper);
            plan_sig = hsh & 0x7fffffffffffffffull;
        }
        if (matched) {
            std::vector<int32_t> rperm((size_t)n);
            for (int32_t k = 0; k < n; k++) rperm[k] = mrow[S.perm[k]];
            HIPC(d_rperm_matched.upload(rperm), ERROR_HIP_MALLOC);
            HIPC(d_cs_matched.upload(dc), ERROR_HIP_MALLOC);
            d_rperm = d_rperm_matched, d_cs = d_cs_matched;
            std::vector<int32_t> dcol((size_t)n);
            for (int32_t j = 0; j < n; j++) dcol[(size_t)mrow[j]] = j;
            HIPC(d_dcol.upload(dcol), ERROR_HIP_MALLOC);
            std::vector<char> seen((size_t)n, 0);
            match_parity = 0;
            for (int32_t i = 0; i < n; i++) {
                if (seen[i]) continue;
                int len = 0;
                for (int32_t j = i; !seen[j]; j = mrow[j]) seen[j] = 1, len++;
                if ((len & 1) == 0) match_parity ^= 1;
            }
            if (opt.complex_pairs) {
                match_parity = 0;
                std::fill(seen.begin(), seen.end(), 0);
                for (int32_t i = 0; i < n / 2; i++) {
                    if (seen[i]) continue;
                    int len = 0;
                    for (int32_t j = i; !seen[j]; j = mrow[2 * j] / 2) seen[j] = 1, len++;
                    if ((len & 1) == 0) match_parity ^= 1;
                }
            }
        }
        lap("perm + signature");
        {
            if (asm_thread.joinable()) asm_thread.join();
            if (opt.verbose) fprintf(stderr, "hipmf: initialize: the assembly-list thread worked %.3f s beside the launch plans\n", AL.seconds);
            if (getenv("HIPMF_PLAN_DIGEST")) {
                uint64_t h = (uint64_t)plan_digest ^ 1469598103934665603ull;
                auto eat = [&](const void *p, size_t bytes) {
                    const unsigned char *b = (const unsigned char *)p;
                    for (size_t i = 0; i < bytes; i++) h = (h ^ b[i]) * 1099511628211ull;
                };
                eat(AL.sa_ptr.data(), AL.sa_ptr.size() * sizeof(int32_t)), eat(AL.sa_k.data(), AL.sa_k.size() * sizeof(int32_t));
                eat(AL.sa_pos.data(), AL.sa_pos.size() * sizeof(AL.sa_pos[0])), eat(AL.sc_k.data(), AL.sc_k.size() * sizeof(int32_t));
                eat(AL.sc_cnt.data(), AL.sc_cnt.size() * sizeof(int64_t)), eat(AL.sc_pos.data(), AL.sc_pos.size() * sizeof(AL.sc_pos[0]));
                eat(AL.ea_sc.data(), AL.ea_sc.size() * sizeof(AL.ea_sc[0]));
                plan_digest = (int64_t)(h & 0x7fffffffffffffffull);
            }
            if (AL.status == 1) {
                last_error = "too many entries in the tiled fronts";
                return ERROR_HIPMF_SYMBOLIC;
            }
            if (AL.status == 2) {
                last_error = "too many zero-fill tasks";
                return ERROR_HIPMF_SYMBOLIC;
            }
            if (AL.status == 3) {
                last_error = "Not enough memory: a host allocation failed";
                return ERROR_MALLOC;
            }
            const int32_t ns = S.nsuper;
            for (int32_t l = 0; l < S.nlevels; l++) {
                levels[(size_t)l].sc_off = (int32_t)AL.sc_cnt[(size_t)l], levels[(size_t)l].sc_cnt = (int32_t)(AL.sc_cnt[(size_t)l + 1] - AL.sc_cnt[(size_t)l]);
                levels[(size_t)l].zero_off = AL.zero_off[(size_t)l], levels[(size_t)l].zero_cnt = AL.zero_n[(size_t)l];
            }
            zero_cnt = AL.zero_cnt;
            HIPC(d_sa_ptr.upload(AL.sa_ptr), ERROR_HIP_MALLOC);
            {
                std::vector<FrontDesc> h_fd((size_t)ns);
                std::vector<int32_t> h_lists((size_t)n_lists);
                HIPC(hipMemcpy(h_fd.data(), d_fd, sizeof(FrontDesc) * (size_t)ns, hipMemcpyDeviceToHost), ERROR_HIP_MEMCPY);
                if (n_lists > 0) HIPC(hipMemcpy(h_lists.data(), d_lists, sizeof(int32_t) * (size_t)n_lists, hipMemcpyDeviceToHost), ERROR_HIP_MEMCPY);
                std::vector<SmallDesc> sd(h_lists.size());
                for (size_t q = 0; q < h_lists.size(); q++) {
                    const int32_t s = h_lists[q];
                    sd[q].fd = h_fd[(size_t)s];
                    sd[q].e0 = AL.sa_ptr[(size_t)s], sd[q].e1 = AL.sa_ptr[(size_t)s + 1];
                }
                HIPC(d_sd.upload(sd), ERROR_HIP_MALLOC);
            }
            HIPC(d_sa_k.upload(AL.sa_k), ERROR_HIP_MALLOC);
            HIPC(d_sa_pos.upload(AL.sa_pos), ERROR_HIP_MALLOC);
            HIPC(d_sc_k.upload(AL.sc_k), ERROR_HIP_MALLOC);
            HIPC(d_sc_at.upload(AL.sc_at), ERROR_HIP_MALLOC);
            if (ea_lds_active()) {
                HIPC(d_ea_sc.upload(AL.ea_sc), ERROR_HIP_MALLOC);
                HIPC(d_sc_pos.upload(AL.sc_pos), ERROR_HIP_MALLOC);
            }
            HIPC(d_zero.upload(AL.zt), ERROR_HIP_MALLOC);
        }
        lap("assembly lists + zero tasks");
        std::vector<int64_t>().swap(S.amap);
        std::vector<int64_t>().swap(S.amap2);
        std::vector<int32_t>().swap(S.amap_sn);
        HIPC(d_vals.alloc(std::max<int64_t>(nnz, 1)), ERROR_HIP_MALLOC);
        HIPC(d_vs.alloc(std::max<int64_t>(nnz, 1)), ERROR_HIP_MALLOC);
        if (sym_lower) HIPC(d_vs2.alloc(std::max<int64_t>(nnz, 1)), ERROR_HIP_MALLOC);
        for (DeviceArray<double> *p : {&d_xp, &d_r, &d_den, &d_b, &d_x, &d_du, &d_rs}) HIPC(p->alloc((size_t)n + WT_X), ERROR_HIP_MALLOC);
        if (matched) HIPC(hipMemcpy(d_rs, dr.data(), sizeof(double) * n, hipMemcpyHostToDevice), ERROR_HIP_MEMCPY);
        HIPC(d_lperm.alloc((size_t)n + WT_X), ERROR_HIP_MALLOC);
        HIPC(hipMemsetAsync(d_lperm, 0, sizeof(int32_t) * ((size_t)n + WT_X), STREAM), ERROR_HIP_MEMCPY);
        for (double *p : {d_xp.get(), d_du.get()}) HIPC(hipMemsetAsync(p + n, 0, sizeof(double) * WT_X, STREAM), ERROR_HIP_MEMCPY);
        HIPC(d_diag.alloc((size_t)n * (opt.complex_pairs ? 2 : 1)), ERROR_HIP_MALLOC);
        if (S.sym_mode) d_cs = d_rs;
        {
            HIPC(hipMalloc((void **)d_info.put(), sizeof(FactorInfoExt)), ERROR_HIP_MALLOC);
            FactorInfoExt ext = {};
            ext.zdiag = opt.complex_pairs ? d_diag + n : nullptr;
            HIPC(hipMemcpy(d_info, &ext, sizeof ext, hipMemcpyHostToDevice), ERROR_HIP_MEMCPY);
        }
        HIPC(d_scalar.alloc(4 + (size_t)RES_NORM_WORDS * SF_KMAX), ERROR_HIP_MALLOC);
        for (EventOwner &e : ev) HIPC(hipEventCreate(e.put()), ERROR_HIP_MALLOC);
        HIPC(hipStreamSynchronize(STREAM), ERROR_HIP_SYNCHRONIZE);
        lap("value / vector buffers");
        return SUCCESSFUL_EXIT;
    };
    const auto t_plan = std::chrono::steady_clock::now();
    int32_t code = upload_plan(tail);
    if (code != SUCCESSFUL_EXIT) return code;
    lap("wait for the solve task lists");
    if (opt.verbose)
        fprintf(stderr,
                "hipmf: initialize: graph %.3f s, ordering %.3f s, etree %.3f s, supernodes %.3f s, row structures %.3f s, layout %.3f s, "
                "assembly map %.3f s; plan + device allocation + upload + tail %.3f s\n",
                S.seconds_phase[0], S.seconds_phase[1], S.seconds_phase[2], S.seconds_phase[3], S.seconds_phase[4], S.seconds_phase[5],
                S.seconds_phase[6], std::chrono::duration<double>(std::chrono::steady_clock::now() - t_plan).count());
    if (opt.verbose) {
        fprintf(stderr, "hipmf: initialize: host pieces:");
        for (const auto &l : laps) fprintf(stderr, " %s %.3f s;", l.first, l.second);
        fprintf(stderr, "\n");
    }
    initialized = true;
    return SUCCESSFUL_EXIT;
}

int32_t Solver::upload_plan(const std::function<int32_t()> &tail) {
    const int32_t ns = S.nsuper;
    block_groups_plan = 8.0 * (double)S.persist_doubles <= block_groups_max_bytes ? SF_GMAX : 1;
    if (const char *e = getenv("HIPMF_BLOCK_GROUPS")) block_groups_plan = std::max(1, std::min((int)SF_GMAX, atoi(e)));
    if (!split_minlen_env) split_minlen = 2048 * block_groups_plan;
    if (!blocked_slabs_env) blocked_slabs = block_groups_plan > 1 && S.max_front >= 16384;
    auto pl_t = std::chrono::steady_clock::now();
    std::string pl_log;
    auto pl_lap = [&](const char *what) {
        const auto now = std::chrono::steady_clock::now();
        char buf[96];
        snprintf(buf, sizeof buf, " %s %.3f s;", what, std::chrono::duration<double>(now - pl_t).count());
        pl_log += buf;
        pl_t = now;
    };
    struct WtPlan {
        bool ok_tree = false;
        std::vector<char> ok;
        std::vector<int32_t> cnt, roots;
        std::vector<int64_t> bytes;
    } WP;
    WP.ok_tree = use_tree && S.n >= 4;
    if (WP.ok_tree) {
        bool tree_ok = true;
        std::vector<char> &ok = WP.ok;
        std::vector<int32_t> &cnt = WP.cnt;
        std::vector<int64_t> &bytes = WP.bytes;
        ok.assign((size_t)ns, 0), cnt.assign((size_t)ns, 0), bytes.assign((size_t)ns, 0);
        std::vector<int32_t> dl((size_t)ns, 0), piv((size_t)ns, 0);
        for (int32_t s = 0; s < ns && tree_ok; s++) {
            const int32_t f = S.fsize(s), p = S.npiv(s);
            bool good = f <= SMALL_F && (int64_t)f * p <= WT_NCH * WT_CHUNK && S.nrow(s) <= WT_MI - 16 * WT_NREC;
            int32_t c = 1, d = 0, pv = p;
            int64_t b = (int64_t)f * p * 8;
            for (int32_t q = S.child_ptr[s]; q < S.child_ptr[s + 1]; q++) {
                const int32_t ch = S.child_idx[q];
                if (ch >= s) tree_ok = false;
                else good = good && ok[(size_t)ch], c += cnt[(size_t)ch], b += bytes[(size_t)ch], d = std::max(d, dl[(size_t)ch]), pv += piv[(size_t)ch];
            }
            if (S.child_ptr[s + 1] > S.child_ptr[s]) d += f;
            cnt[(size_t)s] = c, bytes[(size_t)s] = b, dl[(size_t)s] = d, piv[(size_t)s] = pv;
            ok[(size_t)s] = good && c <= wt_max_fronts && b <= (int64_t)wt_max_kb * 1024 && d <= WT_STACK && pv <= WT_X;
        }
        if (tree_ok) {
            for (int32_t s = 0; s < ns; s++)
                if (ok[(size_t)s] && (S.sn_parent[s] < 0 || !ok[(size_t)S.sn_parent[s]])) WP.roots.push_back(s);
            std::stable_sort(WP.roots.begin(), WP.roots.end(), [&](int32_t a, int32_t b) { return bytes[(size_t)a] > bytes[(size_t)b]; });
            for (size_t ri = 0; ri < WP.roots.size() && tree_ok; ri++) {
                const int32_t R = WP.roots[ri], lo = R - cnt[(size_t)R] + 1;
                for (int32_t s = lo; s < R; s++)
                    if (S.sn_parent[s] < lo || S.sn_parent[s] > R) tree_ok = false;
            }
        }
        WP.ok_tree = tree_ok;
    }
    const bool tag_shape = WP.ok_tree && !WP.roots.empty() && (sf_asm_front <= 0 || S.max_front < sf_asm_front);
    const bool tag_plan = use_tag && tag_shape;
    std::vector<char> interior((size_t)ns, 0);
    if (tag_plan)
        for (int32_t R : WP.roots)
            for (int32_t s = R - WP.cnt[(size_t)R] + 1; s < R; s++) interior[(size_t)s] = 1;
    std::vector<int64_t> woff_of((size_t)ns, 0);
    work_doubles = 0;
    std::vector<char> is_root((size_t)ns, 0);
    if (tag_plan) {
        for (int32_t s = 0; s < ns; s++)
            if (interior[(size_t)s]) woff_of[(size_t)s] = work_doubles, work_doubles += S.fsize(s);
        for (int32_t R : WP.roots) is_root[(size_t)R] = 1, woff_of[(size_t)R] = work_doubles, work_doubles += S.fsize(R);
    }
    work_arm0 = work_doubles;
    for (int32_t s = 0; s < ns; s++)
        if (!interior[(size_t)s] && !is_root[(size_t)s]) woff_of[(size_t)s] = work_doubles, work_doubles += S.fsize(s);
    work_up = work_doubles;
    work_blk_doubles = work_doubles;
    if (tag_plan) work_doubles += S.n;
    std::vector<FrontDesc> fd((size_t)ns);
    for (int32_t s = 0; s < ns; s++) {
        FrontDesc &d = fd[s];
        d.off = S.front_off[s];
        d.rowptr = S.sn_rowptr[s];
        d.woff = woff_of[(size_t)s];
        d.p = S.npiv(s);
        d.m = S.nrow(s);
        d.first = S.sn_first[s];
        d.child_begin = S.child_ptr[s];
        d.child_end = S.child_ptr[s + 1];
        d.parent = S.sn_parent[s];
        d.ld = S.front_ld[s];
        d.ugroup = update_group(S.fsize(s));
        d.eoff = S.e_off[s], d.epoff = S.ep_off[s];
        d.flags = S.fsize(s) > SMALL_F ? (FD_BIG | (S.sym_mode ? FD_SYM : 0) | (is_mid(s) ? FD_DENSE_TOP : 0)) : 0;
        d.ldp = S.front_ldp[s];
    }
    pool_doubles = S.persist_doubles + S.temp_doubles;

    int32_t sp_code = SUCCESSFUL_EXIT;
    auto solve_plans = [&]() -> int32_t {
        std::vector<SfTask> sf;
        std::vector<int32_t> need((size_t)2 * ns, 1);
        std::vector<char> in_w((size_t)ns, 0);
        bool tree = false;
        bool blocked = false;
        bool klist = false;
        int32_t k_fwd_rows = 0;
        int32_t k_bwd_groups = 0;
        int32_t top_level = S.nlevels;
        auto kind_of = [&](int32_t s, bool forward) {
            const int32_t len = forward ? S.npiv(s) : S.fsize(s);
            if (blocked) return forward ? (S.fsize(s) >= sf_big_front || len >= 512 ? 7 : 6) : 6;
            if (!forward && S.sym_mode) return 4;
            if (forward && klist && k_fwd_rows > 0 && S.fsize(s) >= sf_big_front) return k_fwd_rows;
            if (forward && sf_big_rows > 0 && S.fsize(s) >= sf_big_front) return sf_big_rows;
            if (tree && !slab64 && S.sn_level[s] >= top_level) {
                int32_t G = 2;
                while (G < up_max_groups && len > 32 * G) G *= 2;
                return G == 32 ? 3 : (G == 16 ? 4 : (G == 8 ? 5 : (G == 4 ? 6 : 7)));
            }
            if (tree && tag_shape && !forward && !slab64) return len >= mid_bwd_len4 ? 4 : (len >= mid_bwd_len5 ? 5 : (len > 32 ? 6 : 7));
            return slab64 ? 6 : (len >= 512 ? 4 : (len >= 128 ? 5 : (len > 32 ? 6 : 7)));
        };
        bool skip_leaves = false;
        auto is_leaf_front = [&](int32_t s) {
            const int64_t p = S.npiv(s), m = S.nrow(s), f = p + m;
            return S.child_ptr[s + 1] == S.child_ptr[s] && f <= SMALL_F && p >= 1 && p <= LEAF_PMAX && m <= LEAF_MMAX && f * p <= LEAF_PANEL;
        };
        auto emit_level = [&](int32_t l, bool forward) {
            std::vector<int32_t> small, wavef;
            if (klist) {
                k_fwd_rows = 0, k_bwd_groups = 0;
                if (forward && sf_big_rows > 0 && split_tasks > 0) {
                    for (int32_t rows_log = sf_big_rows; rows_log >= 4; rows_log--) {
                        int64_t cnt = 0;
                        for (int32_t k = S.level_ptr[l]; k < S.level_ptr[l + 1]; k++)
                            if (S.fsize(S.level_sn[k]) >= sf_big_front) cnt += (S.fsize(S.level_sn[k]) + (1 << rows_log) - 1) >> rows_log;
                        k_fwd_rows = rows_log;
                        if (cnt == 0 || cnt >= split_tasks) break;
                    }
                    if (k_fwd_rows == sf_big_rows) k_fwd_rows = 0;
                }
                if (!forward)
                    for (int32_t k = S.level_ptr[l]; k < S.level_ptr[l + 1]; k++) {
                        const int32_t s = S.level_sn[k];
                        if (S.fsize(s) > SMALL_F && !(skip_leaves && is_leaf_front(s))) k_bwd_groups += (S.npiv(s) + (1 << kind_of(s, false)) - 1) >> kind_of(s, false);
                    }
            }
            for (int32_t k = S.level_ptr[l]; k < S.level_ptr[l + 1]; k++) {
                int32_t s = S.level_sn[k];
                if (tree && in_w[(size_t)s]) continue;
                if (skip_leaves && is_leaf_front(s)) {
                    need[(size_t)(forward ? 0 : ns) + s] = 0;
                    continue;
                }
                if (S.fsize(s) <= SMALL_F) {
                    small.push_back(s);
                    continue;
                }
                if (tree && forward && wave_fronts && !slab64 && S.sn_level[s] < top_level && S.fsize(s) <= SF_WF_ROWS && S.npiv(s) <= SF_WF_PIV &&
                    S.child_ptr[s + 1] - S.child_ptr[s] <= 64) {
                    wavef.push_back(s);
                    need[(size_t)s] = 1;
                    wave_front_count++;
                    continue;
                }
                if (tree && !forward && wave_fronts && wave_fronts_bwd && !slab64 && !S.sym_mode && S.sn_level[s] < top_level && S.fsize(s) <= SF_WF_ROWS &&
                    S.npiv(s) <= SF_WF_PIV) {
                    wavef.push_back(s);
                    need[(size_t)ns + s] = 1;
                    continue;
                }
                const int32_t kind = kind_of(s, forward), rows = 1 << kind, ext = forward ? S.fsize(s) : S.npiv(s);
                int32_t nasm = 0;
                if (forward && sf_asm_front > 0 && S.fsize(s) >= sf_asm_front && S.child_ptr[s + 1] > S.child_ptr[s] && !(tree && tag_plan)) {
                    for (int32_t q0 = 0; q0 < ext; q0 += SF_ASM_ROWS) sf.push_back({1, s, q0, std::min(ext, q0 + SF_ASM_ROWS), 0, 0}), nasm++;
                }
                need[(size_t)(forward ? 0 : ns) + s] = (ext + rows - 1) / rows + nasm;
                const size_t first_slab = sf.size();
                int32_t Q = 1;
// ... 312 lines not shown
    };
    const bool sp_async = !(getenv("HIPMF_PLAN_THREAD") && atoi(getenv("HIPMF_PLAN_THREAD")) == 0);
    if (!sp_async) sp_code = solve_plans();
    std::thread sp_thread([&]() {
        if (!sp_async) return;
        (void)hipSetDevice(device);
        try {
            sp_code = solve_plans();
        } catch (const std::bad_alloc &) {
            std::lock_guard<std::mutex> lock(err_mutex);
            last_error = "Not enough memory: a host allocation failed";
            sp_code = ERROR_MALLOC;
        }
    });
    struct SpJoiner {
        std::thread &t;
        ~SpJoiner() {
            if (t.joinable()) t.join();
        }
    } sp_joiner{sp_thread};

    std::vector<int32_t> lists, tasks, allbig;
    std::vector<ChainTask> chain;
    chain_words = 0;
    std::vector<FrontDesc> bigfd;
    std::vector<EaTask, NoInitAlloc<EaTask>> ea;
    std::vector<EaRange, NoInitAlloc<EaRange>> ear;
    std::vector<int32_t> tiled_slot((size_t)S.nsuper, -1);
    int32_t max_big = 0;
    std::vector<SolveTask> stasks;
    levels.assign((size_t)S.nlevels, LevelPlan());
    mid_front_count = 0;
    for (int32_t l = 0; l < S.nlevels; l++) {
        LevelPlan &L = levels[l];
        std::vector<int32_t> small, big;
        int32_t fmax_small = 1;
        for (int32_t k = S.level_ptr[l]; k < S.level_ptr[l + 1]; k++) {
            int32_t s = S.level_sn[k];
            if (S.fsize(s) <= SMALL_F) {
                small.push_back(s);
                fmax_small = std::max(fmax_small, S.fsize(s));
                L.small_pmax = std::max(L.small_pmax, S.npiv(s));
            } else {
                big.push_back(s);
            }
        }
        std::vector<int32_t> mid;
        {
            std::vector<int32_t> tiled;
            for (int32_t a : big) (is_mid(a) ? mid : tiled).push_back(a);
            big.swap(tiled);
            auto cls = [&](int32_t a) {
                const int32_t m = S.nrow(a);
                if (!is_mid_lu(a)) return m <= 80 ? 0 : (m <= 128 ? 1 : 2);
                const int32_t w = midl_lds_doubles(S.npiv(a), m);
                return (mid_lu_split && w <= 5000) ? 3 : ((mid_lu_split && w <= 10000) ? 4 : 5);
            };
            std::stable_sort(mid.begin(), mid.end(), [&](int32_t a, int32_t b) {
                return cls(a) != cls(b) ? cls(a) < cls(b) : (int64_t)S.npiv(a) * S.fsize(a) * S.fsize(a) > (int64_t)S.npiv(b) * S.fsize(b) * S.fsize(b);
            });
            mid_front_count += (int64_t)mid.size();
            for (int32_t a : mid) {
                const int c = cls(a);
                L.mid_cnt[c]++;
                L.mid_lds[c] = std::max(L.mid_lds[c], c >= 3 ? midl_lds_doubles(S.npiv(a), S.nrow(a)) : mid_lds_doubles(S.npiv(a), S.nrow(a)));
            }
        }
        std::stable_sort(big.begin(), big.end(), [&](int32_t a, int32_t b) { return S.npiv(a) > S.npiv(b); });
        std::vector<int32_t> mirror;
        if (S.sym_mode)
            for (int32_t a : big)
                if (S.sn_parent[a] >= 0 && S.nrow(a) > 0 && S.fsize(S.sn_parent[a]) <= SMALL_F) mirror.push_back(a);
        std::stable_partition(small.begin(), small.end(), [&](int32_t a) { return S.fsize(a) <= small_split; });
        L.small_cnt_a = 0;
        int32_t fmax_a = 1;
        for (int32_t a : small)
            if (S.fsize(a) <= small_split) L.small_cnt_a++, fmax_a = std::max(fmax_a, S.fsize(a));
        if (L.small_cnt_a < 2048 || (int32_t)small.size() - L.small_cnt_a < 2048) L.small_cnt_a = 0;
        L.small_ld_a = fmax_a | 1;
        L.small_off = (int32_t)lists.size();
        L.small_cnt = (int32_t)small.size();
        L.small_ld = fmax_small | 1;
        lists.insert(lists.end(), small.begin(), small.end());
        L.big_off = (int32_t)lists.size();
        L.big_cnt = (int32_t)big.size();
        lists.insert(lists.end(), big.begin(), big.end());
        L.mirror_off = (int32_t)lists.size();
        L.mirror_cnt = (int32_t)mirror.size();
        lists.insert(lists.end(), mirror.begin(), mirror.end());
        L.bigfd_off = (int32_t)bigfd.size();
        for (int32_t a : big) bigfd.push_back(fd[(size_t)a]);
        L.mid_off = (int32_t)bigfd.size();
        for (int32_t a : mid) bigfd.push_back(fd[(size_t)a]);
        allbig.insert(allbig.end(), big.begin(), big.end());
        max_big = std::max(max_big, L.big_cnt);
        int32_t pmax = big.empty() ? 0 : S.npiv(big[0]);
        {
            int32_t fmax_big = 0;
            for (int32_t a : big) fmax_big = std::max(fmax_big, S.fsize(a));
            const bool forced = getenv("HIPMF_UPD32_MAXF") != nullptr;
            L.upd_ts = (!big.empty() && fmax_big <= upd32_max_front && (!S.sym_mode || forced)) ? UPD_T_SMALL : UPD_T;
        }
        const int64_t UT = L.upd_ts;
        for (int32_t k0 = 0; k0 < pmax; k0 += NB) {
            StepPlan st;
            while (st.nactive < L.big_cnt && S.npiv(big[st.nactive]) > k0) st.nactive++;
            st.pfx_panel = (int64_t)tasks.size();
            int64_t acc = 0;
            for (int32_t a = 0; a < st.nactive; a++) {
                tasks.push_back((int32_t)acc);
                if (a >= 1 && a <= 3) st.ppfx[a - 1] = (int32_t)acc;
                acc += 2 * ((S.fsize(big[a]) + PANEL_T - 1) / PANEL_T);
            }
            tasks.push_back((int32_t)acc);
            st.n_panel = (int32_t)acc;
            st.pfx_update = (int64_t)tasks.size();
            acc = 0;
            for (int32_t a = 0; a < st.nactive; a++) {
                tasks.push_back((int32_t)acc);
                if (a >= 1 && a <= 3) st.upfx[a - 1] = (int32_t)acc;
                const int64_t fa = S.fsize(big[a]), nba = std::min<int64_t>(NB, S.npiv(big[a]) - k0), basea = k0 + nba;
                const int64_t ntF = (fa - basea + UT - 1) / UT, ntE = (basea + UT - 1) / UT;
                int64_t nt = ntF + ntE;
                const bool follow = S.npiv(big[a]) > k0 + NB;
                const int32_t G = update_group(S.fsize(big[a]));
                const bool narrow = follow && ((k0 / NB) % G) != G - 1;
                if (S.sym_mode) acc += (narrow ? nt : ntF * (ntF + 1) / 2 + ntF * ntE) + (follow ? 1 : 0);
                else acc += (narrow ? 2 * nt : nt * nt) + (follow ? 1 : 0);
            }
            tasks.push_back((int32_t)acc);
            if (acc > 0x7fffffffLL) return ERROR_HIPMF_SYMBOLIC;
            st.n_update = (int32_t)acc;
            bool any_narrow = false, any_follow = false, any_full = false;
            for (int32_t a = 0; a < st.nactive; a++) {
                const bool follow = S.npiv(big[a]) > k0 + NB;
                const int32_t G = update_group(S.fsize(big[a]));
                const bool nar = follow && ((k0 / NB) % G) != G - 1;
                any_narrow |= nar, any_follow |= follow, any_full |= !nar;
            }
            st.all_narrow = !any_full;
            if (!S.sym_mode && UT == UPD_T && upd_split_min > 0 && st.n_update >= upd_split_min && !use_chain) {
                if (!any_narrow && any_follow) {
                    st.split = true;
                    for (int part = 1; part <= 2; part++) {
                        (part == 1 ? st.pfx_crit : st.pfx_rest) = (int64_t)tasks.size();
                        int64_t acc2 = 0;
                        for (int32_t a = 0; a < st.nactive; a++) {
                            tasks.push_back((int32_t)acc2);
                            const int64_t fa = S.fsize(big[a]), nba = std::min<int64_t>(NB, S.npiv(big[a]) - k0), basea = k0 + nba;
                            const int64_t nt = (fa - basea + UT - 1) / UT + (basea + UT - 1) / UT;
                            const bool follow = S.npiv(big[a]) > k0 + NB;
                            acc2 += part == 1 ? (2 * nt - 1) + (follow ? 1 : 0) : (nt - 1) * (nt - 1);
                        }
                        tasks.push_back((int32_t)acc2);
                        (part == 1 ? st.n_crit : st.n_rest) = (int32_t)acc2;
                    }
                }
            }
            L.steps.push_back(st);
        }
        L.pfx_flush = (int64_t)tasks.size();
        {
            int64_t accf = 0;
            for (int32_t a : big) {
                tasks.push_back((int32_t)accf);
                const int64_t pa = S.npiv(a);
// ... 472 lines not shown
};
static DeviceGate &device_gate(int device) {
    static DeviceGate gates[64];
    return gates[device >= 0 && device < 64 ? device : 0];
}
struct GateLock {
    DeviceGate &g;
    int device;
    bool owned = false;
    GateLock(DeviceGate &gate, int dev) : g(gate), device(dev) {}
    ~GateLock() {
        if (owned) unlock();
    }
    bool owns_lock() const { return owned; }
    bool lock_counting() {
        bool free_ = g.mu.try_lock();
        if (!free_) g.mu.lock();
        if (!g.file_lock(device)) free_ = false;
        owned = true;
        return free_;
    }
    void lock() { (void)lock_counting(); }
    void unlock() {
        g.file_unlock();
        g.mu.unlock();
        owned = false;
    }
};

int32_t Solver::run_factor() {
    const int32_t n = S.n;
    const int64_t nnz = S.nnz_a;
    int64_t launches = 0;
    HIPC(hipEventRecord((hipEvent_t)ev[0], STREAM), ERROR_HIP_SYNCHRONIZE);
    if (!matched)
        hipLaunchKernelGGL(k_row_scale, dim3((n + 255) / 256), dim3(256), 0, STREAM, n, d_rp, d_vals, d_tptr, d_tidx, opt.scaling, S.sym_mode ? 1 : 0, d_rs);
    HIPC(hipMemsetAsync(d_scalar, 0, 4 * sizeof(unsigned long long), STREAM), ERROR_HIP_MEMCPY);
    HIPC(hipMemsetAsync(d_info, 0, sizeof(FactorInfo), STREAM), ERROR_HIP_MEMCPY);
    const bool chained = use_chain && d_chain_cnt != nullptr;
    GateLock gate(device_gate(device), device);
    if (chained) gate.lock();
    const bool PZ = opt.complex_pairs;
    if (chained) HIPC(hipMemsetAsync(d_chain_cnt, 0, sizeof(int32_t) * (size_t)chain_words, STREAM), ERROR_HIP_MEMCPY);
    int gs = (int)std::min<int64_t>(2048, (nnz + 255) / 256);
    hipLaunchKernelGGL(k_absmax, dim3(gs), dim3(256), 0, STREAM, nnz, d_vals, d_arow, d_ci, d_rs, d_cs, d_vs, d_vs2, d_scalar, d_info);
    launches += 2;
    bool pre_forked = false;
#ifndef HIPMF_EMULATED
    pre_forked = overlap_small && !use_graph && !levels.empty() && levels[0].ea_cnt == 0 && levels[0].steps.empty();
#endif
    hipStream_t pst = STREAM;
    if (pre_forked) {
        HIPC(hipEventRecord((hipEvent_t)ev_pre0, STREAM), ERROR_HIP_SYNCHRONIZE);
        HIPC(hipStreamWaitEvent((hipStream_t)stream4, (hipEvent_t)ev_pre0, 0), ERROR_HIP_SYNCHRONIZE);
        pst = (hipStream_t)stream4;
    }
    const bool sym_first_look = S.sym_lower && opt.matching > 0 && !sym_diag_looked;
    if ((!S.sym_lower && opt.matching > 0) || sym_first_look) {
        hipLaunchKernelGGL(k_diag_check, dim3((n + 255) / 256), dim3(256), 0, pst, n, d_rp, d_ci, d_vs, d_dcol, 0.01, d_info, opt.complex_pairs ? 1 : 0);
        launches++;
    }
    if (zero_cnt > 0) {
        hipLaunchKernelGGL(k_zero, dim3(zero_cnt), dim3(256), 0, pst, d_zero, d_pool);
        hipLaunchKernelGGL(k_set_identity, dim3(allbig_cnt), dim3(256), 0, pst, d_lists + allbig_off, d_fd, d_pool);
        launches += 2;
    }
    if (pre_forked) HIPC(hipEventRecord((hipEvent_t)ev_pre1, (hipStream_t)stream4), ERROR_HIP_SYNCHRONIZE);
    HIPC(hipEventRecord((hipEvent_t)ev[1], STREAM), ERROR_HIP_SYNCHRONIZE);
    auto fill_level = [&](const LevelPlan &L, hipStream_t st) {
        if (L.zero_cnt > 0) {
            hipLaunchKernelGGL(k_zero, dim3(L.zero_cnt), dim3(256), 0, st, d_zero + L.zero_off, d_pool);
            launches++;
        }
        if (L.sc_cnt > 0) {
            hipLaunchKernelGGL(k_scatter, dim3((unsigned)std::min<int64_t>(2048, ((int64_t)L.sc_cnt + 255) / 256)), dim3(256), 0, st, (int64_t)L.sc_cnt,
                               d_sc_k + L.sc_off, d_sc_at + L.sc_off, d_vs, d_vs2, d_pool);
            launches++;
        }
    };
    auto enqueue_levels = [&]() -> int32_t {
    const bool ea_lds = ea_lds_active();
    bool pre_pending = pre_forked;
    if (!levels.empty() && !ea_lds) fill_level(levels[0], STREAM);
    for (size_t li = 0; li < levels.size(); li++) {
        const LevelPlan &L = levels[li];
        const LevelPlan *Lnext = li + 1 < levels.size() ? &levels[li + 1] : nullptr;
        const bool fill_next = !ea_lds && Lnext && (Lnext->zero_cnt > 0 || Lnext->sc_cnt > 0);
        if (pre_pending && (L.ea_cnt > 0 || !L.steps.empty() || L.mid_total() > 0 || fill_next)) {
            HIPC(hipStreamWaitEvent(STREAM, (hipEvent_t)ev_pre1, 0), ERROR_HIP_SYNCHRONIZE);
            pre_pending = false;
        }
        if (L.ea_cnt > 0) {
            if (ea_lds && S.sym_mode)
                hipLaunchKernelGGL(k_extend_add_lds<true>, dim3(L.ea_cnt), dim3(256), sizeof(double) * EA_TILE_C * EA_TILE_R, STREAM, d_ea + L.ea_off, d_ear, d_rel,
                                   d_pool, d_ea_sc + L.ea_off, d_sc_k, d_sc_pos, d_vs, d_vs2, d_dws, d_lperm, d_scalar, opt.pivot_epsilon, d_info, d_diag);
            else if (ea_lds)
                hipLaunchKernelGGL((PZ ? k_extend_add_lds<false, true> : k_extend_add_lds<false, false>), dim3(L.ea_cnt), dim3(256), sizeof(double) * EA_TILE_C * EA_TILE_R, STREAM, d_ea + L.ea_off, d_ear, d_rel,
                                   d_pool, d_ea_sc + L.ea_off, d_sc_k, d_sc_pos, d_vs, d_vs2, d_dws, d_lperm, d_scalar, opt.pivot_epsilon, d_info, d_diag);
            else if (S.sym_mode) hipLaunchKernelGGL(k_extend_add<true>, dim3(L.ea_cnt), dim3(256), 0, STREAM, d_ea + L.ea_off, d_ear, d_rel, d_pool);
            else hipLaunchKernelGGL(k_extend_add<false>, dim3(L.ea_cnt), dim3(256), 0, STREAM, d_ea + L.ea_off, d_ear, d_rel, d_pool);
            launches++;
        }
        const bool has_mid = L.mid_total() > 0;
        const bool forked = overlap_small && ((L.small_cnt > 0 && (!L.steps.empty() || has_mid)) || fill_next);
        if (L.small_cnt > 0) {
            size_t shmem = sizeof(double) * (size_t)L.small_ld * (size_t)L.small_ld;
            hipStream_t sst = STREAM;
            if (forked) {
                HIPC(hipEventRecord((hipEvent_t)ev_fork, STREAM), ERROR_HIP_SYNCHRONIZE);
                HIPC(hipStreamWaitEvent((hipStream_t)stream2, (hipEvent_t)ev_fork, 0), ERROR_HIP_SYNCHRONIZE);
                sst = (hipStream_t)stream2;
            }
            const SmallAsm sasm = {d_sd, d_sa_k, d_sa_pos, d_vs, d_vs2, d_child, d_rel, d_lists};
            const bool pair = small_pair && L.small_cnt_a > 0 && !forked && !use_graph && L.steps.empty() && !has_mid;
            if (L.small_cnt_a > 0) {
                const size_t shmem_a = sizeof(double) * (size_t)L.small_ld_a * (size_t)L.small_ld_a;
                hipStream_t ast = sst;
                if (pair) {
                    HIPC(hipEventRecord((hipEvent_t)ev_fork3, STREAM), ERROR_HIP_SYNCHRONIZE);
                    HIPC(hipStreamWaitEvent((hipStream_t)stream3, (hipEvent_t)ev_fork3, 0), ERROR_HIP_SYNCHRONIZE);
                    ast = (hipStream_t)stream3;
                }
                hipLaunchKernelGGL((PZ ? k_small_factor<1, true> : k_small_factor<1, false>), dim3(L.small_cnt_a), dim3(64), shmem_a, ast, d_lists + L.small_off, d_fd, d_pool, d_lperm,
                                   d_scalar, opt.pivot_epsilon, d_info, L.small_ld_a, sasm, d_diag);
                launches++;
                if (pair) HIPC(hipEventRecord((hipEvent_t)ev_join3, (hipStream_t)stream3), ERROR_HIP_SYNCHRONIZE);
            }
            const int32_t cnt_b = L.small_cnt - L.small_cnt_a;
            if (cnt_b <= small_wide_max && L.small_ld > 33)
                hipLaunchKernelGGL((PZ ? k_small_factor<4, true> : k_small_factor<4, false>), dim3(cnt_b), dim3(256), shmem, sst, d_lists + L.small_off + L.small_cnt_a, d_fd, d_pool, d_lperm,
                                   d_scalar, opt.pivot_epsilon, d_info, L.small_ld, sasm, d_diag);
            else
                hipLaunchKernelGGL((PZ ? k_small_factor<1, true> : k_small_factor<1, false>), dim3(cnt_b), dim3(64), shmem, sst, d_lists + L.small_off + L.small_cnt_a, d_fd, d_pool, d_lperm,
                                   d_scalar, opt.pivot_epsilon, d_info, L.small_ld, sasm, d_diag);
            launches++;
            if (pair) HIPC(hipStreamWaitEvent(STREAM, (hipEvent_t)ev_join3, 0), ERROR_HIP_SYNCHRONIZE);
        } else if (forked) {
            HIPC(hipEventRecord((hipEvent_t)ev_fork, STREAM), ERROR_HIP_SYNCHRONIZE);
            HIPC(hipStreamWaitEvent((hipStream_t)stream2, (hipEvent_t)ev_fork, 0), ERROR_HIP_SYNCHRONIZE);
        }
        if (fill_next) fill_level(*Lnext, forked ? (hipStream_t)stream2 : STREAM);
        if (forked) HIPC(hipEventRecord((hipEvent_t)ev_join, (hipStream_t)stream2), ERROR_HIP_SYNCHRONIZE);
        const bool mid_forked = overlap_small && has_mid && (!L.steps.empty() || forked);
        if (has_mid) {
            hipStream_t mst = STREAM;
            if (mid_forked) {
                if (forked) HIPC(hipStreamWaitEvent((hipStream_t)stream3, (hipEvent_t)ev_fork, 0), ERROR_HIP_SYNCHRONIZE);
                else {
                    HIPC(hipEventRecord((hipEvent_t)ev_fork3, STREAM), ERROR_HIP_SYNCHRONIZE);
                    HIPC(hipStreamWaitEvent((hipStream_t)stream3, (hipEvent_t)ev_fork3, 0), ERROR_HIP_SYNCHRONIZE);
                }
                mst = (hipStream_t)stream3;
            }
            int32_t moff = L.mid_off;
            for (int c = LevelPlan::MID_CLASSES - 1; c >= 0; c--) moff += L.mid_cnt[c];
            for (int c = LevelPlan::MID_CLASSES - 1; c >= 0; c--) {
                moff -= L.mid_cnt[c];
                if (L.mid_cnt[c] == 0) continue;
                const size_t dyn = sizeof(double) * (size_t)L.mid_lds[c];
                const FrontDesc *mfd = d_bigfd + moff;
                if (c >= 3) {
                    hipLaunchKernelGGL((PZ ? k_front_lu<true> : k_front_lu<false>), dim3(L.mid_cnt[c]), dim3(64 * MIDL_NW), dyn, mst, mfd, d_pool, d_lperm, d_scalar, opt.pivot_epsilon, d_info, d_diag);
                    launches++;
                    continue;
                }
#define HIPMF_LAUNCH_FRONT(CM) \
    hipLaunchKernelGGL(k_front<CM>, dim3(L.mid_cnt[c]), dim3(64 * MID_NW), dyn, mst, mfd, d_pool, d_lperm, d_scalar, opt.pivot_epsilon, d_info, d_diag)
                if (c == 0) HIPMF_LAUNCH_FRONT(10);
                else if (c == 1) HIPMF_LAUNCH_FRONT(16);
                else HIPMF_LAUNCH_FRONT(24);
#undef HIPMF_LAUNCH_FRONT
                launches++;
            }
            if (mid_forked) {
                if (forked) HIPC(hipStreamWaitEvent((hipStream_t)stream3, (hipEvent_t)ev_join, 0), ERROR_HIP_SYNCHRONIZE);
                HIPC(hipEventRecord((hipEvent_t)ev_join3, (hipStream_t)stream3), ERROR_HIP_SYNCHRONIZE);
            }
        }
        int32_t k0 = 0;
        if (chained && L.chain_cnt > 0) {
            const FrontDesc *lfd = d_bigfd + L.bigfd_off;
            const StepPlan &st0 = L.steps[0];
            const int32_t pre_lu = 1;
            if (pre_lu) {
                if (S.sym_mode) hipLaunchKernelGGL(k_diag0<true>, dim3(st0.nactive), dim3(64), 0, STREAM, lfd, d_pool, d_lperm, d_dws, d_scalar, opt.pivot_epsilon, d_info, d_diag);
                else hipLaunchKernelGGL((PZ ? k_diag0<false, true> : k_diag0<false, false>), dim3(st0.nactive), dim3(64), 0, STREAM, lfd, d_pool, d_lperm, d_dws, d_scalar, opt.pivot_epsilon, d_info, d_diag);
                launches++;
            }
            const ChainTask *ct = (const ChainTask *)d_chain + L.chain_off;
            if (S.sym_mode)
                hipLaunchKernelGGL(k_chain<true>, dim3(L.chain_cnt), dim3(256), 0, STREAM, ct, lfd, d_pool, d_lperm, d_dws, dws_stride, d_scalar,
                                   opt.pivot_epsilon, d_info, d_diag, pre_lu, d_chain_cnt, d_chain_cnt + (chain_words - 1));
            else
                hipLaunchKernelGGL(k_chain<false>, dim3(L.chain_cnt), dim3(256), 0, STREAM, ct, lfd, d_pool, d_lperm, d_dws, dws_stride, d_scalar,
                                   opt.pivot_epsilon, d_info, d_diag, pre_lu, d_chain_cnt, d_chain_cnt + (chain_words - 1));
            launches++;
        } else {
        bool rest_pending = false;
        for (const StepPlan &st : L.steps) {
            const FrontDesc *lfd = d_bigfd + L.bigfd_off;
            const bool ea_lu = ea_lu_active();
            const int32_t pre_lu = (k0 == 0 && (ea_lu || (st.n_panel >= diag0_min_panels && (S.sym_mode || !use_binv)))) ? 1 : 0;
            if (pre_lu && !ea_lu) {
                if (S.sym_mode) hipLaunchKernelGGL(k_diag0<true>, dim3(st.nactive), dim3(64), 0, STREAM, lfd, d_pool, d_lperm, d_dws, d_scalar, opt.pivot_epsilon, d_info, d_diag);
                else hipLaunchKernelGGL((PZ ? k_diag0<false, true> : k_diag0<false, false>), dim3(st.nactive), dim3(64), 0, STREAM, lfd, d_pool, d_lperm, d_dws, d_scalar, opt.pivot_epsilon, d_info, d_diag);
                launches++;
            }
            if (S.sym_mode) {
                hipLaunchKernelGGL(k_panel<true>, dim3(st.n_panel), dim3(PANEL_T), 0, STREAM, d_tasks + st.pfx_panel, st.nactive, lfd, k0,
                                   d_pool, d_lperm, d_dws, dws_stride, d_scalar, opt.pivot_epsilon, d_info, d_diag, pre_lu, Pfx4{st.ppfx[0], st.ppfx[1], st.ppfx[2]});
                if (st.n_update > 0 && L.upd_ts == UPD_T)
                    hipLaunchKernelGGL(k_update<true>, dim3(st.n_update), dim3(256), 0, STREAM, d_tasks + st.pfx_update, st.nactive, lfd, k0,
                                       d_pool, d_dws, dws_stride, d_lperm, d_scalar, opt.pivot_epsilon, d_info, d_diag, 0, Pfx4{st.upfx[0], st.upfx[1], st.upfx[2]});
                else if (st.n_update > 0)
                    hipLaunchKernelGGL(k_update32<true>, dim3(st.n_update), dim3(64), 0, STREAM, d_tasks + st.pfx_update, st.nactive, lfd, k0,
                                       d_pool, d_dws, dws_stride, d_lperm, d_scalar, opt.pivot_epsilon, d_info, d_diag, Pfx4{st.upfx[0], st.upfx[1], st.upfx[2]});
            } else if (use_binv) {
// ... 2027 lines not shown
```

russell_amd/csrc/numeric.hpp:

```cpp
#pragma once
#include <cstdint>
#include <functional>
#include <mutex>
#include <string>
#include <vector>

#include "device_owner.hpp"
#include "symbolic.hpp"

namespace hipmf {

struct FrontDesc;
struct SmallDesc;
struct EaTask;
struct EaRange;
struct SolveTask;
struct SfTask;
struct WtHdr;
struct WtWave;
struct LeafRec;
struct ZeroTask;
struct FactorInfo;

enum : int32_t {
    SUCCESSFUL_EXIT = 0,
    ERROR_NULL_POINTER = 100000,
    ERROR_MALLOC = 200000,
    ERROR_VERSION = 300000,
    ERROR_NOT_AVAILABLE = 400000,
    ERROR_NEED_INITIALIZATION = 500000,
    ERROR_NEED_FACTORIZATION = 600000,
    ERROR_ALREADY_INITIALIZED = 700000,
    ERROR_HIP_MALLOC = 100,
    ERROR_HIP_MEMCPY = 200,
    ERROR_HIP_SYNCHRONIZE = 300,
    ERROR_HIP_LAUNCH = 350,
    ERROR_HIPMF_INVALID_MATRIX = 600,
    ERROR_HIPMF_SYMBOLIC = 700,
    ERROR_HIPMF_INVALID_VALUE = 803,
    ERROR_HIPMF_COMM = 900,
    ERROR_HIPMF_NO_DEVICE = 1000,
    WARNING_SINGULAR_MATRIX = 1,
};

struct NumericOptions {
    int32_t scaling = 1;
    double pivot_epsilon = 1e-13;
    int32_t refinement_nstep = 2;
    int32_t matching = 1;
    double device_memory_factor = 0.0;
    bool complex_pairs = false;
    bool verbose = false;
};

struct PhaseTimes {
    double scale_assemble_ms = 0, factor_ms = 0, fwd_ms = 0, bwd_ms = 0, solve_total_ms = 0;
    int64_t n_kernel_launches_factor = 0, n_kernel_launches_solve = 0;
    double acc_factor_ms = 0, acc_assemble_ms = 0, acc_fwd_ms = 0, acc_bwd_ms = 0;
    int64_t acc_factor_count = 0, acc_tri_count = 0;
};

struct StepPlan {
    int32_t nactive = 0;
    int64_t pfx_panel = 0, pfx_update = 0;
    int32_t n_panel = 0, n_update = 0;
    int32_t ppfx[3] = {0x7fffffff, 0x7fffffff, 0x7fffffff}, upfx[3] = {0x7fffffff, 0x7fffffff, 0x7fffffff};
    bool split = false;
    bool all_narrow = false;
    int64_t pfx_crit = 0, pfx_rest = 0;
    int32_t n_crit = 0, n_rest = 0;
};
struct LevelPlan {
    int32_t small_off = 0, small_cnt = 0, small_ld = 0, small_pmax = 1;
    int32_t small_cnt_a = 0, small_ld_a = 1;
    int32_t big_off = 0, big_cnt = 0;
    int32_t bigfd_off = 0;
    int32_t ea_off = 0, ea_cnt = 0;
    int32_t mirror_off = 0, mirror_cnt = 0;
    int32_t zero_off = 0, zero_cnt = 0;
    int32_t sc_off = 0, sc_cnt = 0;
    int32_t fwd_off = 0, fwd_cnt = 0, bwd_off = 0, bwd_cnt = 0;
    int32_t big_pmax = 0, big_fmax = 0;
    bool wide = false;
    std::vector<StepPlan> steps;
    int64_t pfx_flush = 0;
    int32_t n_flush = 0;
    int32_t upd_ts = 64;
    int32_t mid_off = 0;
    static constexpr int MID_CLASSES = 6;
    int32_t mid_cnt[MID_CLASSES] = {0, 0, 0, 0, 0, 0};
    int32_t mid_lds[MID_CLASSES] = {0, 0, 0, 0, 0, 0};
    int32_t mid_total() const {
        int32_t t = 0;
        for (int c = 0; c < MID_CLASSES; c++) t += mid_cnt[c];
        return t;
    }
    int64_t chain_off = 0;
    int32_t chain_cnt = 0;
};

struct ChainTask;

struct SolverTransposed {
    struct TrLevel {
        int32_t small_off = 0, small_cnt = 0, asm_off = 0, asm_cnt = 0, gf_off = 0, gf_cnt = 0, ga_off = 0, ga_cnt = 0, gb_off = 0, gb_cnt = 0;
        int32_t small_pmax = 1, small_fmax = 1;
    };
    std::vector<TrLevel> tr_levels;
    bool tr_ready = false;
    DeviceArray<int32_t> d_tr_list, d_ttptr, d_ttrow, d_ttmap;
    DeviceArray<SolveTask> d_tr_tasks;
    DeviceArray<double> d_work_t, d_tvec;
    DeviceArray<double> d_anl;
    DeviceArray<unsigned long long> d_tnrm;
    PinnedArray<double> h_tnrm;
    bool tr_blk_ready = false;
    DeviceArray<double> d_work_tb, d_tblk;
    DeviceArray<unsigned long long> d_tnrm_blk;
    PinnedArray<double> h_tnrm_blk;
};

struct SolverPruned {
    struct SpLevel {
        int32_t small_off = 0, small_cnt = 0, pmax = 1, fmax = 1;
        int32_t va_off = 0, va_cnt = 0;
        int32_t pr_off = 0, pr_cnt = 0;
    };
    template <class T> struct Growing {
        DeviceArray<T> a;
        size_t cap = 0;
        hipError_t need(size_t count) {
            if (count <= cap) return hipSuccess;
            const hipError_t e = a.alloc(count + count / 2 + 64);
            cap = e == hipSuccess ? count + count / 2 + 64 : 0;
            return e;
        }
    };
    bool sp_ready = false;
    std::vector<int32_t> sp_ipos_r, sp_ipos_c;
    std::vector<int32_t> sp_stamp_f, sp_stamp_b;
    int32_t sp_epoch = 0;
    double sp_total_pf = 0.0;
    DeviceArray<int32_t> d_sp_ipos_r, d_sp_ipos_c, d_sp_mark;
    DeviceArray<double> d_sp_xp, d_sp_work;
    Growing<int32_t> d_sp_fwd, d_sp_bwd, d_sp_idx, d_sp_sel;
    Growing<double> d_sp_val, d_sp_out, d_sp_dense;
    EventOwner sp_ev0, sp_ev1;
};

struct SolverDevice : SolverTransposed, SolverPruned {
    DeviceArray<double> d_pool;
    DeviceArray<int32_t> d_lperm;
    DeviceArray<double> d_rs;
    DeviceArray<double> d_cs_matched;
    double *d_cs = nullptr;
    DeviceArray<int32_t> d_rperm_matched;
    int32_t *d_rperm = nullptr;
    DeviceArray<int32_t> d_dcol;
    DeviceArray<LeafRec> d_leaf;
    int32_t leaf_cnt = 0;
    int64_t split_units = 0;
    int64_t split_slabs = 0;
    DeviceArray<double> d_split_scr;
    DeviceArray<int32_t> d_split_cnt;
    DeviceArray<SfTask> d_sfk;
    DeviceArray<int32_t> d_needk;
    DeviceArray<SfTask> d_sf3;
    DeviceArray<int32_t> d_need3;
    DeviceArray<FrontDesc> d_fd;
    DeviceArray<FrontDesc> d_bigfd;
    DeviceArray<EaTask> d_ea;
    DeviceArray<EaRange> d_ear;
    DeviceArray<double> d_dws;
    DeviceArray<SolveTask> d_st;
    DeviceArray<SfTask> d_sf;
    DeviceArray<WtHdr> d_wt_hdr;
    DeviceArray<int32_t> d_wt_meta;
    DeviceArray<WtWave> d_wt_wave;
    int32_t wt_waves = 0, wt_recs = 0;
    DeviceArray<SfTask> d_sf2;
    int32_t sf2_fwd_cnt = 0, sf2_bwd_cnt = 0;
    DeviceArray<int32_t> d_rep_idx;
    DeviceArray<int32_t> d_rep;
    int64_t rep_words = 0;
    DeviceArray<int32_t> d_need2;
    DeviceArray<int32_t> d_need;
    DeviceArray<int32_t> d_sync;
    DeviceArray<ChainTask> d_chain;
    DeviceArray<int32_t> d_chain_cnt;
    int64_t chain_words = 0;
    DeviceArray<int32_t> d_sa_ptr, d_sa_k;
    DeviceArray<uint16_t> d_sa_pos;
    DeviceArray<ZeroTask> d_zero;
    DeviceArray<double> d_vs, d_vs2;
    int32_t zero_cnt = 0;
    DeviceArray<int32_t> d_seg_ptr, d_seg_idx;
    DeviceArray<int32_t> d_emap;
    DeviceArray<double> d_vlow;
    int64_t nnz_low = 0;
    DeviceArray<double> d_vin;
    int64_t nnz_in = 0;
    DeviceArray<SmallDesc> d_sd;
    DeviceArray<double> d_blk, d_work_blk;
    DeviceArray<unsigned long long> d_norms_blk;
    int32_t block_cols = 0;
    int32_t block_groups = 0;
    DeviceArray<unsigned long long> d_trace;
    DeviceArray<FactorInfo> d_info;
    DeviceArray<unsigned long long> d_scalar;
    DeviceArray<double> d_work, d_vals, d_xp, d_r, d_den, d_b, d_x, d_du;
    DeviceArray<int32_t> d_rows, d_rel, d_child, d_lists, d_tasks;
    DeviceArray<int32_t> d_rp, d_ci, d_arow, d_tptr, d_tidx, d_perm;
    DeviceArray<int32_t> d_ea_sc;
    DeviceArray<uint16_t> d_sc_pos;
    DeviceArray<int32_t> d_sc_k;
    DeviceArray<int64_t> d_sc_at;
    DeviceArray<double> d_diag;
    DeviceArray<int32_t> d_row_blk;
    struct LaneBuffers {
        StreamOwner stream;
        DeviceArray<double> blk, work;
        DeviceArray<int32_t> sync;
        DeviceArray<unsigned long long> norms;
    };
    std::vector<LaneBuffers> extra_lanes;
    PinnedArray<double> h_nrm;
    PinnedArray<double> h_stage;
#ifndef HIPMF_EMULATED
    GraphExecOwner factor_graph;
#endif
    int64_t graph_launches = 0;
    EventOwner ev[8];
    EventOwner ev_fork, ev_join;
    EventOwner ev_pb, ev_rest;
    EventOwner ev_pre0, ev_pre1;
    EventOwner ev_fork3, ev_join3;
    StreamOwner stream;
    StreamOwner stream2;
    StreamOwner stream3;
    StreamOwner stream4;
};

class Solver : public SolverDevice {
  public:
    Solver();
    ~Solver();
    int32_t initialize(int32_t n, const int32_t *rp, const int32_t *ci, bool sym_lower, const SymbolicOptions &sopt,
                       const NumericOptions &nopt, const double *values = nullptr);
    int32_t factorize(const double *values, bool on_device);
    int32_t set_value_map(int64_t nnz_in, const int32_t *seg_ptr, const int32_t *seg_idx, bool signed_map = false);
    int32_t factorize_mapped(const double *input, bool on_device);
    int32_t solve(double *x, const double *rhs, int32_t nrhs, int64_t ldx, bool on_device);
    int32_t solve_core(double *x, const double *rhs, int32_t nrhs, int64_t ldx, bool on_device);
    struct KrylovOps {
        std::function<int32_t(double *, const double *)> precond, apply;
    };
    int32_t krylov_rescue(double *x, const double *rhs, bool on_device, const KrylovOps *ops = nullptr);
    int32_t solve_transpose(double *x, const double *rhs, int32_t nrhs, int64_t ldx, bool on_device, bool conj_pairs = false);
    int32_t solve_transpose_many(double *x, const double *rhs, int32_t nrhs, int64_t ldx, bool on_device);
    int64_t transposed_blocks = 0;
    int32_t error_analysis(const double *xbar, const double *rhs, double *out, int32_t option);
    int32_t error_analysis_complex(const double *xbar, const double *rhs, double *out, int32_t option);
// ... 192 lines not shown
```

Baseline: 7.175 ms.

## Factor whole small-front subtrees in one workgroup with an LDS contribution stack

Adds a subtree factorisation kernel in which a single 64-lane workgroup walks a postordered chain of small fronts. For each front it assembles the original entries, extend-adds the children's contribution blocks from an LDS stack, runs the LU and stores the factors, so those fronts leave the per-level small-factor launches. The aim is to remove per-level launches and the global-memory round trips of small contribution blocks in the lower elimination tree. The costs are one-wave-per-subtree serialisation, limited parallelism for deep subtrees, and LDS pressure from the class sizes, which could lower occupancy. It is enabled by default.

```diff
diff --git a/include/russell_hipmf.h b/include/russell_hipmf.h
--- a/include/russell_hipmf.h
+++ b/include/russell_hipmf.h
@@ -140,6 +140,10 @@
 #define HIPMF_COUNTER_PRUNED_BWD_FRONTS 25
 #define HIPMF_COUNTER_PRUNED_BLOCKS 26
 #define HIPMF_COUNTER_PRUNED_BYTES 27
+#define HIPMF_COUNTER_SUBTREE_FACTOR_FRONTS 28
+#define HIPMF_COUNTER_SUBTREE_FACTOR_CUTS 29
+#define HIPMF_COUNTER_SUBTREE_ROOTS_UNDER_MID 30
+#define HIPMF_COUNTER_SUBTREE_ROOTS_UNDER_TILED 31
 int64_t solver_hipmf_get_counter(struct InterfaceHIPMF *solver, int32_t which);
 
 #define HIPMF_OPTION_MATCHING 0
@@ -185,6 +189,7 @@
 int32_t complex_solver_hipmf_factorize_mapped(struct InterfaceComplexHIPMF *solver, int32_t *effective_ordering, int32_t *effective_scaling,
                                               int32_t *num_perturbed_pivots, double *rcond_estimate, C_BOOL verbose, const double *input_values);
 int32_t complex_solver_hipmf_get_stats(struct InterfaceComplexHIPMF *solver, int64_t *istats, double *dstats);
+int32_t complex_solver_hipmf_factor_parts(struct InterfaceComplexHIPMF *solver, int32_t max_parts, void **d_ptrs, int64_t *bytes);
 int64_t complex_solver_hipmf_get_counter(struct InterfaceComplexHIPMF *solver, int32_t which);
 const char *complex_solver_hipmf_last_error(struct InterfaceComplexHIPMF *solver);
 
diff --git a/russell_amd/_capi.py b/russell_amd/_capi.py
--- a/russell_amd/_capi.py
+++ b/russell_amd/_capi.py
@@ -59,6 +59,7 @@
                                                            C.POINTER(C.c_double), C.c_int32, f64p]),
     "complex_solver_hipmf_get_stats": (C.c_int32, [C.c_void_p, i64p, f64p]),
     "complex_solver_hipmf_get_counter": (C.c_int64, [C.c_void_p, C.c_int32]),
+    "complex_solver_hipmf_factor_parts": (C.c_int32, [C.c_void_p, C.c_int32, C.POINTER(C.c_void_p), C.POINTER(C.c_int64)]),
     "complex_solver_hipmf_last_error": (C.c_char_p, [C.c_void_p]),
     "solver_hipmf_get_counter": (C.c_int64, [C.c_void_p, C.c_int32]),
     "solver_hipmf_set_option": (C.c_int32, [C.c_void_p, C.c_int32, C.c_double]),
diff --git a/russell_amd/backend.py b/russell_amd/backend.py
--- a/russell_amd/backend.py
+++ b/russell_amd/backend.py
@@ -176,7 +176,7 @@
         out.update({k: float(v) for k, v in zip(DSTAT_NAMES, d)})
         return out
 
-    COUNTERS = {"rematch": 0, "weak_diagonal_rows": 1, "fused_fallbacks": 2, "persistent_bytes": 3, "arena_bytes": 4, "symmetric_ldlt": 5, "sym_expanded": 6, "chain_fallbacks": 7, "mid_fronts": 8, "plan_digest": 9, "tagged_solve": 10, "gate_waits": 11, "wave_fronts": 12, "leaf_fronts": 13, "split_slabs": 14, "event_fence_free": 15, "block_groups": 16, "sym_weak_diagonal": 17, "bcast_sliced_bytes": 18, "krylov_iterations": 19, "transposed_solves": 20, "analysis_solves": 21, "transposed_krylov_iterations": 22, "transposed_blocks": 23, "pruned_fwd_fronts": 24, "pruned_bwd_fronts": 25, "pruned_blocks": 26, "pruned_bytes": 27}
+    COUNTERS = {"rematch": 0, "weak_diagonal_rows": 1, "fused_fallbacks": 2, "persistent_bytes": 3, "arena_bytes": 4, "symmetric_ldlt": 5, "sym_expanded": 6, "chain_fallbacks": 7, "mid_fronts": 8, "plan_digest": 9, "tagged_solve": 10, "gate_waits": 11, "wave_fronts": 12, "leaf_fronts": 13, "split_slabs": 14, "event_fence_free": 15, "block_groups": 16, "sym_weak_diagonal": 17, "bcast_sliced_bytes": 18, "krylov_iterations": 19, "transposed_solves": 20, "analysis_solves": 21, "transposed_krylov_iterations": 22, "transposed_blocks": 23, "pruned_fwd_fronts": 24, "pruned_bwd_fronts": 25, "pruned_blocks": 26, "pruned_bytes": 27, "subtree_factor_fronts": 28, "subtree_factor_cuts": 29, "subtree_roots_under_mid": 30, "subtree_roots_under_tiled": 31}
 
     OPTIONS = {"matching": 0, "pivoting": 1, "hybrid_memory": 2, "error_estimates": 3, "condition_numbers": 4, "sym_recheck": 5}
 
diff --git a/russell_amd/csrc/interface_complex_hipmf.cpp b/russell_amd/csrc/interface_complex_hipmf.cpp
--- a/russell_amd/csrc/interface_complex_hipmf.cpp
+++ b/russell_amd/csrc/interface_complex_hipmf.cpp
@@ -317,6 +317,17 @@
     return guarded(h, [&]() { return c_get_stats_body(h, is, ds); });
 }
 
+int32_t complex_solver_hipmf_factor_parts(struct InterfaceComplexHIPMF *h, int32_t max_parts, void **d_ptrs, int64_t *bytes) {
+    if (!h || !d_ptrs || !bytes) return ERROR_NULL_POINTER;
+    if (!h->solver.initialized) return ERROR_NEED_INITIALIZATION;
+    if (max_parts < 4) return ERROR_HIPMF_INVALID_VALUE;
+    const Solver &s = h->solver;
+    void *p[4] = {s.d_pool, s.d_lperm, s.d_rs, s.d_diag_ptr()};
+    const int64_t nb[4] = {s.S.persist_doubles * 8, (int64_t)s.S.n * 4, (int64_t)s.S.n * 8, (int64_t)s.S.n * 8 * (s.opt.complex_pairs ? 2 : 1)};
+    for (int i = 0; i < 4; i++) d_ptrs[i] = p[i], bytes[i] = nb[i];
+    return 4;
+}
+
 int64_t complex_solver_hipmf_get_counter(struct InterfaceComplexHIPMF *h, int32_t which) {
     if (!h || !h->solver.initialized) return -1;
     const Solver &s = h->solver;
@@ -338,6 +349,10 @@
     case HIPMF_COUNTER_TRANSPOSED_SOLVES: return s.transposed_solves;
     case HIPMF_COUNTER_ANALYSIS_SOLVES: return s.analysis_solves;
     case HIPMF_COUNTER_TRANSPOSED_KRYLOV_ITERATIONS: return s.krylov_iterations_t;
+    case HIPMF_COUNTER_SUBTREE_FACTOR_FRONTS: return s.stf_fronts;
+    case HIPMF_COUNTER_SUBTREE_FACTOR_CUTS: return s.stf_cut;
+    case HIPMF_COUNTER_SUBTREE_ROOTS_UNDER_MID: return s.stf_roots_mid;
+    case HIPMF_COUNTER_SUBTREE_ROOTS_UNDER_TILED: return s.stf_roots_tiled;
     default: return -1;
     }
 }
diff --git a/russell_amd/csrc/interface_hipmf.cpp b/russell_amd/csrc/interface_hipmf.cpp
--- a/russell_amd/csrc/interface_hipmf.cpp
+++ b/russell_amd/csrc/interface_hipmf.cpp
@@ -588,6 +588,10 @@
     case HIPMF_COUNTER_PRUNED_BWD_FRONTS: return s.pruned_bwd_fronts;
     case HIPMF_COUNTER_PRUNED_BLOCKS: return s.pruned_blocks;
     case HIPMF_COUNTER_PRUNED_BYTES: return s.pruned_bytes;
+    case HIPMF_COUNTER_SUBTREE_FACTOR_FRONTS: return s.stf_fronts;
+    case HIPMF_COUNTER_SUBTREE_FACTOR_CUTS: return s.stf_cut;
+    case HIPMF_COUNTER_SUBTREE_ROOTS_UNDER_MID: return s.stf_roots_mid;
+    case HIPMF_COUNTER_SUBTREE_ROOTS_UNDER_TILED: return s.stf_roots_tiled;
     default: return -1;
     }
 }
diff --git a/russell_amd/csrc/kernels.hpp b/russell_amd/csrc/kernels.hpp
--- a/russell_amd/csrc/kernels.hpp
+++ b/russell_amd/csrc/kernels.hpp
@@ -2,6 +2,7 @@
 #include "kernels_assembly.hpp"
 #include "kernels_common.hpp"
 #include "kernels_factor.hpp"
+#include "kernels_factor_subtree.hpp"
 #include "kernels_extend_add.hpp"
 #include "kernels_factor_front.hpp"
 #include "kernels_factor_binv.hpp"
diff --git a/russell_amd/csrc/kernels_factor.hpp b/russell_amd/csrc/kernels_factor.hpp
--- a/russell_amd/csrc/kernels_factor.hpp
+++ b/russell_amd/csrc/kernels_factor.hpp
@@ -180,6 +180,32 @@
     const int32_t *list0;
 };
 
+template <int NW>
+__device__ __forceinline__ void small_front_store(const double *sm, const int ld, const int f, const int p, double *__restrict__ F,
+                                                  double *__restrict__ Up, const int32_t *lp, int32_t *__restrict__ lperm_f,
+                                                  double *__restrict__ diag_f) {
+    const int tid = threadIdx.x & 63, grp = threadIdx.x >> 6;
+    const bool split = Up != nullptr;
+    if (tid < f) {
+        int c = grp;
+        for (; c + 7 * NW < f; c += 8 * NW) {
+            double a[8];
+#pragma unroll
+            for (int q = 0; q < 8; q++) a[q] = sm[tid + (c + q * NW) * ld];
+#pragma unroll
+            for (int q = 0; q < 8; q++) F[tid + (c + q * NW) * f] = (split && c + q * NW < p && tid <= c + q * NW) ? 0.0 : a[q];
+        }
+        for (; c < f; c += NW) F[tid + c * f] = (split && c < p && tid <= c) ? 0.0 : sm[tid + c * ld];
+    }
+    if (split && tid < p) {
+        for (int c = grp; c < f; c += NW) Up[tid + c * p] = (tid > c) ? 0.0 : sm[tid + c * ld];
+    }
+    if (grp == 0 && tid < p) {
+        lperm_f[tid] = lp[tid];
+        diag_f[tid] = sm[tid + tid * ld];
+    }
+}
+
 template <int NW, bool PAIRED = false>
 __global__ void __launch_bounds__(64 * NW, NW == 1 ? 6 : 2) k_small_factor(const int32_t *__restrict__ list, const FrontDesc *__restrict__ FD,
                                                           double *__restrict__ pool, int32_t *__restrict__ lperm,
@@ -270,26 +296,7 @@
     __syncthreads();
     if constexpr (PAIRED) lds_lu_blocked<NW, true, true>(sm, ld, f, p, lp, pivpos, eps, rep, info, reinterpret_cast<const FactorInfoExt *>(info)->zdiag + fd.first);
     else lds_lu_blocked<NW, true>(sm, ld, f, p, lp, pivpos, eps, rep, info);
-    const bool split = fd.epoff >= 0;
-    if (tid < f) {
-        int c = grp;
-        for (; c + 7 * NW < f; c += 8 * NW) {
-            double a[8];
-#pragma unroll
-            for (int q = 0; q < 8; q++) a[q] = sm[tid + (c + q * NW) * ld];
-#pragma unroll
-            for (int q = 0; q < 8; q++) F[tid + (c + q * NW) * f] = (split && c + q * NW < p && tid <= c + q * NW) ? 0.0 : a[q];
-        }
-        for (; c < f; c += NW) F[tid + c * f] = (split && c < p && tid <= c) ? 0.0 : sm[tid + c * ld];
-    }
-    if (split && tid < p) {
-        double *Up = pool + fd.epoff;
-        for (int c = grp; c < f; c += NW) Up[tid + c * p] = (tid > c) ? 0.0 : sm[tid + c * ld];
-    }
-    if (grp == 0 && tid < p) {
-        lperm[fd.first + tid] = lp[tid];
-        diag[fd.first + tid] = sm[tid + tid * ld];
-    }
+    small_front_store<NW>(sm, ld, f, p, F, fd.epoff >= 0 ? pool + fd.epoff : nullptr, lp, lperm + fd.first, diag + fd.first);
 }
 
 template <bool PIVOT = true, bool PAIRED = false>
diff --git a/russell_amd/csrc/kernels_factor_subtree.hpp b/russell_amd/csrc/kernels_factor_subtree.hpp
--- /dev/null
+++ b/russell_amd/csrc/kernels_factor_subtree.hpp
@@ -0,0 +1,137 @@
+#pragma once
+#include "kernels_factor.hpp"
+
+namespace hipmf {
+
+constexpr int STF_DEPTH = 64;
+constexpr int STF_ECHUNKS = 2;
+
+struct StfRec {
+    int64_t off;
+    int64_t epoff;
+    int64_t relptr;
+    int32_t pm;
+    int32_t first;
+    int32_t e0, e1;
+    int32_t nch;
+    int32_t pad[5];
+};
+static_assert(sizeof(StfRec) == 64, "16 words");
+
+struct StfWave {
+    int32_t rec0, nrec;
+    int32_t ld;
+    int32_t fa;
+};
+
+struct StfAsm {
+    const int32_t *sa_k;
+    const uint16_t *sa_pos;
+    const double *vs, *vs2;
+    const int32_t *rel;
+};
+
+template <bool PAIRED>
+__global__ void __launch_bounds__(64) k_subtree_factor(const StfWave *__restrict__ waves, const int32_t *__restrict__ recs, double *__restrict__ pool,
+                                                       int32_t *__restrict__ lperm, const unsigned long long *__restrict__ anorm_bits,
+                                                       double pivot_eps, FactorInfo *info, StfAsm A, double *__restrict__ diag) {
+    HIPMF_DYN_SHARED(double, sm);
+    __shared__ int32_t lp[SMALL_F];
+    __shared__ int32_t pivpos[LU_KB];
+    __shared__ int32_t st_off[STF_DEPTH], st_m[STF_DEPTH];
+    const int lane = threadIdx.x;
+    const StfWave w = waves[blockIdx.x];
+    const int ld = w.ld, nrec = w.nrec;
+    double *ST = sm + w.fa;
+    const double eps = pivot_eps * __longlong_as_double((long long)*anorm_bits);
+    const double rep = pivot_replacement(pivot_eps, __longlong_as_double((long long)*anorm_bits));
+    const int32_t *R = recs + 16 * (int64_t)w.rec0;
+    int rc = R[lane & 15];
+    int rn = R[16 * (1 < nrec ? 1 : 0) + (lane & 15)];
+    int kkc[STF_ECHUNKS], posc[STF_ECHUNKS];
+    double vc[STF_ECHUNKS];
+    {
+        const int e0 = wave_bcast_i32(rc, 8), e1 = wave_bcast_i32(rc, 9);
+#pragma unroll
+        for (int c = 0; c < STF_ECHUNKS; c++) {
+            const int e = e0 + 64 * c + lane;
+            kkc[c] = e < e1 ? A.sa_k[e] : 0;
+            posc[c] = e < e1 ? A.sa_pos[e] : 0;
+        }
+#pragma unroll
+        for (int c = 0; c < STF_ECHUNKS; c++) vc[c] = (e0 + 64 * c + lane < e1) ? (kkc[c] < 0 ? A.vs2[~kkc[c]] : A.vs[kkc[c]]) : 0.0;
+    }
+    int sp = 0, top = 0;
+    for (int q = 0; q < nrec; q++) {
+        const int64_t off = (int64_t)(((unsigned long long)(unsigned)wave_bcast_i32(rc, 1) << 32) | (unsigned)wave_bcast_i32(rc, 0));
+        const int64_t epoff = (int64_t)(((unsigned long long)(unsigned)wave_bcast_i32(rc, 3) << 32) | (unsigned)wave_bcast_i32(rc, 2));
+        const int64_t relptr = (int64_t)(((unsigned long long)(unsigned)wave_bcast_i32(rc, 5) << 32) | (unsigned)wave_bcast_i32(rc, 4));
+        const int pm = wave_bcast_i32(rc, 6), first = wave_bcast_i32(rc, 7);
+        const int e0 = wave_bcast_i32(rc, 8), e1 = wave_bcast_i32(rc, 9), nch = wave_bcast_i32(rc, 10);
+        const int p = pm & 0xffff, m = pm >> 16, f = p + m;
+        const bool last = q + 1 >= nrec;
+        const int rn2 = R[16 * (q + 2 < nrec ? q + 2 : nrec - 1) + (lane & 15)];
+        const int e0n = last ? 0 : wave_bcast_i32(rn, 8), e1n = last ? 0 : wave_bcast_i32(rn, 9);
+        int kkn[STF_ECHUNKS], posn[STF_ECHUNKS];
+#pragma unroll
+        for (int c = 0; c < STF_ECHUNKS; c++) {
+            const int e = e0n + 64 * c + lane;
+            kkn[c] = e < e1n ? A.sa_k[e] : 0;
+            posn[c] = e < e1n ? A.sa_pos[e] : 0;
+        }
+        const int myrel = (!last && lane < m) ? A.rel[relptr + lane] : 0;
+        for (int e = lane; e < f * ld; e += 64) sm[e] = 0.0;
+        __syncthreads();
+#pragma unroll
+        for (int c = 0; c < STF_ECHUNKS; c++)
+            if (e0 + 64 * c + lane < e1) sm[(posc[c] & 255) + (posc[c] >> 8) * ld] = vc[c];
+        for (int e = e0 + 64 * STF_ECHUNKS + lane; e < e1; e += 64) {
+            const int kk = A.sa_k[e];
+            const int pos = A.sa_pos[e];
+            sm[(pos & 255) + (pos >> 8) * ld] = kk < 0 ? A.vs2[~kk] : A.vs[kk];
+        }
+        __syncthreads();
+        for (int ci = sp - nch; ci < sp; ci++) {
+            const int mc = wave_uniform(st_m[ci]);
+            if (mc == 0) continue;
+            const double *CB = ST + wave_uniform(st_off[ci]);
+            const int32_t *crel = reinterpret_cast<const int32_t *>(CB + mc * mc);
+            const int sh = mc <= 16 ? 4 : (mc <= 32 ? 5 : 6);
+            const int i = lane & ((1 << sh) - 1), g = lane >> sh, G = 64 >> sh;
+            const int ri = i < mc ? crel[i] : 0;
+            for (int jb = 0; jb < mc; jb += G) {
+                const int j = jb + g;
+                const int rj = __shfl(ri, j & 63);
+                if (i < mc && j < mc) sm[ri + rj * ld] += CB[i + j * mc];
+            }
+            wave_sync();
+        }
+        if (nch > 0) {
+            top = wave_uniform(st_off[sp - nch]);
+            sp -= nch;
+        }
+        if (lane < p) lp[lane] = lane;
+        __syncthreads();
+        if constexpr (PAIRED) lds_lu_blocked<1, true, true>(sm, ld, f, p, lp, pivpos, eps, rep, info, reinterpret_cast<const FactorInfoExt *>(info)->zdiag + first);
+        else lds_lu_blocked<1, true>(sm, ld, f, p, lp, pivpos, eps, rep, info);
+        double vn[STF_ECHUNKS];
+#pragma unroll
+        for (int c = 0; c < STF_ECHUNKS; c++) vn[c] = (e0n + 64 * c + lane < e1n) ? (kkn[c] < 0 ? A.vs2[~kkn[c]] : A.vs[kkn[c]]) : 0.0;
+        small_front_store<1>(sm, ld, f, p, pool + off, epoff >= 0 ? pool + epoff : nullptr, lp, lperm + first, diag + first);
+        if (!last) {
+            double *CB = ST + top;
+            if (lane < m)
+                for (int c = 0; c < m; c++) CB[lane + c * m] = sm[(p + lane) + (p + c) * ld];
+            if (lane < m) reinterpret_cast<int32_t *>(CB + m * m)[lane] = myrel;
+            if (lane == 0) st_off[sp] = top, st_m[sp] = m;
+            sp++;
+            top += m * m + ((m + 1) >> 1);
+            __syncthreads();
+        }
+        rc = rn, rn = rn2;
+#pragma unroll
+        for (int c = 0; c < STF_ECHUNKS; c++) kkc[c] = kkn[c], posc[c] = posn[c], vc[c] = vn[c];
+    }
+}
+
+}
diff --git a/russell_amd/csrc/numeric.cpp b/russell_amd/csrc/numeric.cpp
--- a/russell_amd/csrc/numeric.cpp
+++ b/russell_amd/csrc/numeric.cpp
@@ -253,6 +253,13 @@
     if (const char *e = getenv("HIPMF_OVERLAP_SMALL")) overlap_small = atoi(e) != 0;
     small_pair = false;
     if (const char *e = getenv("HIPMF_SMALL_PAIR")) small_pair = atoi(e) != 0;
+    if (const char *e = getenv("HIPMF_SUBTREE_FACTOR")) use_subtree_factor = atoi(e) != 0;
+    if (const char *e = getenv("HIPMF_SUBTREE_LDS_KB")) stf_lds_kb = std::max(1, std::min(64, atoi(e)));
+    if (const char *e = getenv("HIPMF_SUBTREE_CLASSES")) {
+        int a[STF_CLASSES];
+        if (sscanf(e, "%d,%d,%d,%d", &a[0], &a[1], &a[2], &a[3]) == 4 && a[0] >= 1 && a[0] <= a[1] && a[1] <= a[2] && a[2] <= a[3] && a[3] <= 64)
+            for (int c = 0; c < STF_CLASSES; c++) stf_cls_kb[c] = a[c];
+    }
     if (const char *e = getenv("HIPMF_TREE_SOLVE")) use_tree = atoi(e) != 0;
     if (const char *e = getenv("HIPMF_TAG_SOLVE")) use_tag = atoi(e) != 0;
     if (const char *e = getenv("HIPMF_LEAF_KERNELS")) leaf_kernels = atoi(e) != 0;
@@ -671,6 +678,12 @@
                     sd[q].e0 = AL.sa_ptr[(size_t)s], sd[q].e1 = AL.sa_ptr[(size_t)s + 1];
                 }
                 HIPC(d_sd.upload(sd), ERROR_HIP_MALLOC);
+                for (size_t q = 0; q < stf_rec_sn.size(); q++) {
+                    const int32_t s = stf_rec_sn[q];
+                    stf_rec_host[16 * q + 8] = AL.sa_ptr[(size_t)s], stf_rec_host[16 * q + 9] = AL.sa_ptr[(size_t)s + 1];
+                }
+                if (!stf_rec_host.empty()) HIPC(d_stf_rec.upload(stf_rec_host), ERROR_HIP_MALLOC);
+                std::vector<int32_t>().swap(stf_rec_host), std::vector<int32_t>().swap(stf_rec_sn);
             }
             HIPC(d_sa_k.upload(AL.sa_k), ERROR_HIP_MALLOC);
             HIPC(d_sa_pos.upload(AL.sa_pos), ERROR_HIP_MALLOC);
@@ -821,6 +834,88 @@
         d.ldp = S.front_ldp[s];
     }
     pool_doubles = S.persist_doubles + S.temp_doubles;
+
+    std::vector<char> in_stf((size_t)ns, 0);
+    stf_rec_host.clear(), stf_rec_sn.clear();
+    stf_fronts = stf_cut = stf_roots_mid = stf_roots_tiled = 0;
+    for (int c = 0; c < STF_CLASSES; c++) stf_cls_off[c] = stf_cls_cnt[c] = stf_cls_lds[c] = 0;
+    d_stf_wave.reset(), d_stf_rec.reset();
+    if (use_subtree_factor && WP.ok_tree && !WP.roots.empty()) {
+        struct Sub {
+            int32_t lo, R, ld, fa, lds, cls;
+        };
+        std::vector<Sub> subs;
+        const int64_t cap = std::min<int64_t>((int64_t)stf_lds_kb, stf_cls_kb[STF_CLASSES - 1]) * 1024 / 8;
+        auto measure = [&](int32_t lo, int32_t R, Sub &out) -> bool {
+            int32_t fmax = 1;
+            for (int32_t s = lo; s <= R; s++) fmax = std::max(fmax, S.fsize(s));
+            const int32_t ld = fmax | 1;
+            int64_t top = 0, peak = 0;
+            std::vector<int64_t> sz;
+            for (int32_t s = lo; s <= R; s++) {
+                const int32_t nch = S.child_ptr[s + 1] - S.child_ptr[s];
+                if ((int32_t)sz.size() < nch) return false;
+                for (int32_t k = 0; k < nch; k++) {
+                    if (S.child_idx[S.child_ptr[s] + k] < lo || (k > 0 && S.child_idx[S.child_ptr[s] + k] <= S.child_idx[S.child_ptr[s] + k - 1])) return false;
+                }
+                for (int32_t k = 0; k < nch; k++) top -= sz.back(), sz.pop_back();
+                if (s == R) break;
+                const int64_t m = S.nrow(s), z = m * m + (m + 1) / 2;
+                sz.push_back(z), top += z;
+                peak = std::max(peak, top);
+                if ((int32_t)sz.size() > STF_DEPTH) return false;
+            }
+            const int64_t fa = (int64_t)fmax * ld, lds = fa + peak;
+            if (lds > cap) return false;
+            out.lo = lo, out.R = R, out.ld = ld, out.fa = (int32_t)fa, out.lds = (int32_t)lds, out.cls = 0;
+            while (out.cls < STF_CLASSES - 1 && lds * 8 > (int64_t)stf_cls_kb[out.cls] * 1024) out.cls++;
+            return true;
+        };
+        std::vector<int32_t> todo;
+        for (int32_t R0 : WP.roots) {
+            todo.assign(1, R0);
+            while (!todo.empty()) {
+                const int32_t R = todo.back();
+                todo.pop_back();
+                Sub sb;
+                if (measure(R - WP.cnt[(size_t)R] + 1, R, sb)) {
+                    subs.push_back(sb);
+                    continue;
+                }
+                stf_cut++;
+                for (int32_t q = S.child_ptr[R]; q < S.child_ptr[R + 1]; q++) todo.push_back(S.child_idx[q]);
+            }
+        }
+        std::stable_sort(subs.begin(), subs.end(), [](const Sub &a, const Sub &b) { return a.cls > b.cls; });
+        std::vector<StfWave> wv;
+        for (const Sub &sb : subs) {
+            StfWave w;
+            w.rec0 = (int32_t)stf_rec_sn.size(), w.nrec = sb.R - sb.lo + 1, w.ld = sb.ld, w.fa = sb.fa;
+            const int c = STF_CLASSES - 1 - sb.cls;
+            if (stf_cls_cnt[c] == 0) stf_cls_off[c] = (int32_t)wv.size();
+            stf_cls_cnt[c]++, stf_cls_lds[c] = std::max(stf_cls_lds[c], sb.lds);
+            wv.push_back(w);
+            if (const int32_t par = S.sn_parent[sb.R]; par >= 0 && S.fsize(par) > SMALL_F) (is_mid(par) ? stf_roots_mid : stf_roots_tiled)++;
+            for (int32_t t = sb.lo; t <= sb.R; t++) {
+                StfRec r;
+                memset(&r, 0, sizeof r);
+                r.off = fd[(size_t)t].off, r.epoff = fd[(size_t)t].epoff, r.relptr = fd[(size_t)t].rowptr;
+                r.pm = S.npiv(t) | (S.nrow(t) << 16), r.first = S.sn_first[t];
+                r.nch = S.child_ptr[t + 1] - S.child_ptr[t];
+                const size_t at = stf_rec_host.size();
+                stf_rec_host.resize(at + 16);
+                memcpy(stf_rec_host.data() + at, &r, sizeof r);
+                stf_rec_sn.push_back(t);
+                in_stf[(size_t)t] = 1, stf_fronts++;
+            }
+        }
+        if (!wv.empty()) HIPC(d_stf_wave.upload(wv), ERROR_HIP_MALLOC);
+        if (opt.verbose) {
+            fprintf(stderr, "hipmf: initialize: subtree factorisation: %lld of %d fronts in %zu subtrees (%lld cut);", (long long)stf_fronts, ns, wv.size(), (long long)stf_cut);
+            for (int c = 0; c < STF_CLASSES; c++) fprintf(stderr, " %d x %d B", stf_cls_cnt[c], 8 * stf_cls_lds[c]);
+            fprintf(stderr, "; roots below one-workgroup / tiled fronts: %lld / %lld\n", (long long)stf_roots_mid, (long long)stf_roots_tiled);
+        }
+    }
 
     int32_t sp_code = SUCCESSFUL_EXIT;
     auto solve_plans = [&]() -> int32_t {
@@ -1299,6 +1394,21 @@
         L.small_cnt = (int32_t)small.size();
         L.small_ld = fmax_small | 1;
         lists.insert(lists.end(), small.begin(), small.end());
+        L.fs_off = L.small_off, L.fs_cnt = L.small_cnt, L.fs_ld = L.small_ld, L.fs_cnt_a = L.small_cnt_a, L.fs_ld_a = L.small_ld_a;
+        if (stf_fronts > 0) {
+            std::vector<int32_t> rest;
+            int32_t fmax_r = 1, fmax_ra = 1;
+            L.fs_cnt_a = 0;
+            for (int32_t a : small) {
+                if (in_stf[(size_t)a]) continue;
+                rest.push_back(a), fmax_r = std::max(fmax_r, S.fsize(a));
+                if (S.fsize(a) <= small_split) L.fs_cnt_a++, fmax_ra = std::max(fmax_ra, S.fsize(a));
+            }
+            if (L.fs_cnt_a < 2048 || (int32_t)rest.size() - L.fs_cnt_a < 2048) L.fs_cnt_a = 0;
+            L.fs_ld_a = fmax_ra | 1;
+            L.fs_off = (int32_t)lists.size(), L.fs_cnt = (int32_t)rest.size(), L.fs_ld = fmax_r | 1;
+            lists.insert(lists.end(), rest.begin(), rest.end());
+        }
         L.big_off = (int32_t)lists.size();
         L.big_cnt = (int32_t)big.size();
         lists.insert(lists.end(), big.begin(), big.end());
@@ -1937,6 +2047,15 @@
     const bool ea_lds = ea_lds_active();
     bool pre_pending = pre_forked;
     if (!levels.empty() && !ea_lds) fill_level(levels[0], STREAM);
+    if (stf_fronts > 0) {
+        const StfAsm sa = {d_sa_k, d_sa_pos, d_vs, d_vs2, d_rel};
+        for (int c = 0; c < STF_CLASSES; c++) {
+            if (stf_cls_cnt[c] == 0) continue;
+            hipLaunchKernelGGL((PZ ? k_subtree_factor<true> : k_subtree_factor<false>), dim3(stf_cls_cnt[c]), dim3(64), sizeof(double) * (size_t)stf_cls_lds[c], STREAM,
+                               d_stf_wave + stf_cls_off[c], d_stf_rec, d_pool, d_lperm, d_scalar, opt.pivot_epsilon, d_info, sa, d_diag);
+            launches++;
+        }
+    }
     for (size_t li = 0; li < levels.size(); li++) {
         const LevelPlan &L = levels[li];
         const LevelPlan *Lnext = li + 1 < levels.size() ? &levels[li + 1] : nullptr;
@@ -1957,9 +2076,9 @@
             launches++;
         }
         const bool has_mid = L.mid_total() > 0;
-        const bool forked = overlap_small && ((L.small_cnt > 0 && (!L.steps.empty() || has_mid)) || fill_next);
-        if (L.small_cnt > 0) {
-            size_t shmem = sizeof(double) * (size_t)L.small_ld * (size_t)L.small_ld;
+        const bool forked = overlap_small && ((L.fs_cnt > 0 && (!L.steps.empty() || has_mid)) || fill_next);
+        if (L.fs_cnt > 0) {
+            size_t shmem = sizeof(double) * (size_t)L.fs_ld * (size_t)L.fs_ld;
             hipStream_t sst = STREAM;
             if (forked) {
                 HIPC(hipEventRecord((hipEvent_t)ev_fork, STREAM), ERROR_HIP_SYNCHRONIZE);
@@ -1967,27 +2086,27 @@
                 sst = (hipStream_t)stream2;
             }
             const SmallAsm sasm = {d_sd, d_sa_k, d_sa_pos, d_vs, d_vs2, d_child, d_rel, d_lists};
-            const bool pair = small_pair && L.small_cnt_a > 0 && !forked && !use_graph && L.steps.empty() && !has_mid;
-            if (L.small_cnt_a > 0) {
-                const size_t shmem_a = sizeof(double) * (size_t)L.small_ld_a * (size_t)L.small_ld_a;
+            const bool pair = small_pair && L.fs_cnt_a > 0 && !forked && !use_graph && L.steps.empty() && !has_mid;
+            if (L.fs_cnt_a > 0) {
+                const size_t shmem_a = sizeof(double) * (size_t)L.fs_ld_a * (size_t)L.fs_ld_a;
                 hipStream_t ast = sst;
                 if (pair) {
                     HIPC(hipEventRecord((hipEvent_t)ev_fork3, STREAM), ERROR_HIP_SYNCHRONIZE);
                     HIPC(hipStreamWaitEvent((hipStream_t)stream3, (hipEvent_t)ev_fork3, 0), ERROR_HIP_SYNCHRONIZE);
                     ast = (hipStream_t)stream3;
                 }
-                hipLaunchKernelGGL((PZ ? k_small_factor<1, true> : k_small_factor<1, false>), dim3(L.small_cnt_a), dim3(64), shmem_a, ast, d_lists + L.small_off, d_fd, d_pool, d_lperm,
-                                   d_scalar, opt.pivot_epsilon, d_info, L.small_ld_a, sasm, d_diag);
+                hipLaunchKernelGGL((PZ ? k_small_factor<1, true> : k_small_factor<1, false>), dim3(L.fs_cnt_a), dim3(64), shmem_a, ast, d_lists + L.fs_off, d_fd, d_pool, d_lperm,
+                                   d_scalar, opt.pivot_epsilon, d_info, L.fs_ld_a, sasm, d_diag);
                 launches++;
                 if (pair) HIPC(hipEventRecord((hipEvent_t)ev_join3, (hipStream_t)stream3), ERROR_HIP_SYNCHRONIZE);
             }
-            const int32_t cnt_b = L.small_cnt - L.small_cnt_a;
-            if (cnt_b <= small_wide_max && L.small_ld > 33)
-                hipLaunchKernelGGL((PZ ? k_small_factor<4, true> : k_small_factor<4, false>), dim3(cnt_b), dim3(256), shmem, sst, d_lists + L.small_off + L.small_cnt_a, d_fd, d_pool, d_lperm,
-                                   d_scalar, opt.pivot_epsilon, d_info, L.small_ld, sasm, d_diag);
+            const int32_t cnt_b = L.fs_cnt - L.fs_cnt_a;
+            if (cnt_b <= small_wide_max && L.fs_ld > 33)
+                hipLaunchKernelGGL((PZ ? k_small_factor<4, true> : k_small_factor<4, false>), dim3(cnt_b), dim3(256), shmem, sst, d_lists + L.fs_off + L.fs_cnt_a, d_fd, d_pool, d_lperm,
+                                   d_scalar, opt.pivot_epsilon, d_info, L.fs_ld, sasm, d_diag);
             else
-                hipLaunchKernelGGL((PZ ? k_small_factor<1, true> : k_small_factor<1, false>), dim3(cnt_b), dim3(64), shmem, sst, d_lists + L.small_off + L.small_cnt_a, d_fd, d_pool, d_lperm,
-                                   d_scalar, opt.pivot_epsilon, d_info, L.small_ld, sasm, d_diag);
+                hipLaunchKernelGGL((PZ ? k_small_factor<1, true> : k_small_factor<1, false>), dim3(cnt_b), dim3(64), shmem, sst, d_lists + L.fs_off + L.fs_cnt_a, d_fd, d_pool, d_lperm,
+                                   d_scalar, opt.pivot_epsilon, d_info, L.fs_ld, sasm, d_diag);
             launches++;
             if (pair) HIPC(hipStreamWaitEvent(STREAM, (hipEvent_t)ev_join3, 0), ERROR_HIP_SYNCHRONIZE);
         } else if (forked) {
diff --git a/russell_amd/csrc/numeric.hpp b/russell_amd/csrc/numeric.hpp
--- a/russell_amd/csrc/numeric.hpp
+++ b/russell_amd/csrc/numeric.hpp
@@ -18,6 +18,7 @@
 struct SfTask;
 struct WtHdr;
 struct WtWave;
+struct StfWave;
 struct LeafRec;
 struct ZeroTask;
 struct FactorInfo;
@@ -73,6 +74,7 @@
 struct LevelPlan {
     int32_t small_off = 0, small_cnt = 0, small_ld = 0, small_pmax = 1;
     int32_t small_cnt_a = 0, small_ld_a = 1;
+    int32_t fs_off = 0, fs_cnt = 0, fs_ld = 0, fs_cnt_a = 0, fs_ld_a = 1;
     int32_t big_off = 0, big_cnt = 0;
     int32_t bigfd_off = 0;
     int32_t ea_off = 0, ea_cnt = 0;
@@ -178,6 +180,16 @@
     DeviceArray<int32_t> d_wt_meta;
     DeviceArray<WtWave> d_wt_wave;
     int32_t wt_waves = 0, wt_recs = 0;
+    static constexpr int STF_CLASSES = 4;
+    DeviceArray<StfWave> d_stf_wave;
+    DeviceArray<int32_t> d_stf_rec;
+    std::vector<int32_t> stf_rec_host, stf_rec_sn;
+    int32_t stf_cls_off[STF_CLASSES] = {0, 0, 0, 0}, stf_cls_cnt[STF_CLASSES] = {0, 0, 0, 0}, stf_cls_lds[STF_CLASSES] = {0, 0, 0, 0};
+    int64_t stf_fronts = 0, stf_cut = 0;
+    int64_t stf_roots_mid = 0, stf_roots_tiled = 0;
+    bool use_subtree_factor = true;
+    int32_t stf_lds_kb = 64;
+    int32_t stf_cls_kb[STF_CLASSES] = {8, 16, 32, 64};
     DeviceArray<SfTask> d_sf2;
     int32_t sf2_fwd_cnt = 0, sf2_bwd_cnt = 0;
     DeviceArray<int32_t> d_rep_idx;
```

After: 8.106 ms. 13.0% more time.
